# PorousMediaSimulation/openLBMPM

Measured on AMD Instinct MI355X. Metric: MLUPS (million lattice updates/s), higher is better.
Workload: dtype f64

## Files before the change

### include/lbmpm.h

```cpp
#ifndef LBMPM_H
#define LBMPM_H

#include <stddef.h>
#include <stdint.h>

#ifdef __cplusplus
extern "C" {
#endif

typedef enum lbmpm_status {
    LBMPM_OK = 0,
    LBMPM_ERR_INVALID = -1,
    LBMPM_ERR_HIP = -2,
    LBMPM_ERR_NOMEM = -3,
    LBMPM_ERR_STATE = -4,
    LBMPM_ERR_UNSUPPORTED = -5,
    LBMPM_ERR_TIMEOUT = -6
} lbmpm_status;

const char *lbmpm_last_error(void);
const char *lbmpm_version(void);
int lbmpm_device_count(void);
int lbmpm_hbm_stream_test(int device, int64_t bytes_per_buffer, int reps, double *copy_gbs, double *read_gbs, double *inplace_gbs);

// ... 126 lines not shown
int lbmpm_sc2d_create(const lbmpm_sc2d_config *cfg, const uint8_t *is_domain, lbmpm_sc2d **out);
void lbmpm_sc2d_destroy(lbmpm_sc2d *ctx);
int lbmpm_sc2d_set_pdf(lbmpm_sc2d *ctx, const double *pdf0, const double *pdf1);
int lbmpm_sc2d_set_density(lbmpm_sc2d *ctx, const double *rho0, const double *rho1);
int lbmpm_sc2d_step(lbmpm_sc2d *ctx, int64_t nsteps);
int lbmpm_sc2d_step_timed(lbmpm_sc2d *ctx, int64_t nsteps, double *ms_total, double *ms_dominant);
int lbmpm_sc2d_sync(lbmpm_sc2d *ctx);
int lbmpm_sc2d_enable_diagnostics(lbmpm_sc2d *ctx, int on);
int lbmpm_sc2d_get_field(lbmpm_sc2d *ctx, int field, double *out);
int64_t lbmpm_sc2d_num_fluid_nodes(const lbmpm_sc2d *ctx);
int64_t lbmpm_sc2d_steps_done(const lbmpm_sc2d *ctx);
const char *lbmpm_sc2d_dominant_kernel(const lbmpm_sc2d *ctx);
int64_t lbmpm_sc2d_device_bytes(const lbmpm_sc2d *ctx);

typedef struct lbmpm_rk3d_config {
    int64_t nx, ny, nz_local, nz_global, z_offset;
    double ak_r, ak_b;
    double beta;
    double tau_r, tau_b;
    double solid_phi;
    double inlet_vz_r, inlet_vz_b;
    double outlet_rho_r, outlet_rho_b;
    int32_t device;
    int32_t variant;
    int32_t relaxation;
    int32_t inlet_type;
    double recolor_axis, recolor_diag;
    double inlet_rho_r, inlet_rho_b;
    int32_t outlet_type;
    int32_t reserved;
} lbmpm_rk3d_config;

typedef struct lbmpm_rk3d lbmpm_rk3d;

enum { LBMPM_RK3D_PHI = 0, LBMPM_RK3D_RHO_R = 1, LBMPM_RK3D_RHO_B = 2, LBMPM_RK3D_VX = 3,
       LBMPM_RK3D_VY = 4, LBMPM_RK3D_VZ = 5 };
enum { LBMPM_RK3D_BUF_F_SEND_UP = 0, LBMPM_RK3D_BUF_F_SEND_DOWN = 1,
       LBMPM_RK3D_BUF_F_RECV_FROM_BELOW = 2, LBMPM_RK3D_BUF_F_RECV_FROM_ABOVE = 3,
       LBMPM_RK3D_BUF_PHI_SEND_UP = 4, LBMPM_RK3D_BUF_PHI_SEND_DOWN = 5,
       LBMPM_RK3D_BUF_PHI_RECV_FROM_BELOW = 6, LBMPM_RK3D_BUF_PHI_RECV_FROM_ABOVE = 7 };

int lbmpm_rk3d_create(const lbmpm_rk3d_config *cfg, const uint8_t *is_domain_with_halo, lbmpm_rk3d **out);
void lbmpm_rk3d_destroy(lbmpm_rk3d *ctx);
int lbmpm_rk3d_set_stream(lbmpm_rk3d *ctx, void *hip_stream);
int lbmpm_rk3d_set_density(lbmpm_rk3d *ctx, const double *rho_r, const double *rho_b);
int lbmpm_rk3d_set_macro(lbmpm_rk3d *ctx, const double *rho_r, const double *rho_b, const double *vx, const double *vy, const double *vz);
int lbmpm_rk3d_set_pdf(lbmpm_rk3d *ctx, const double *pdf_r, const double *pdf_b, int post_collision);
int lbmpm_rk3d_get_pdf(lbmpm_rk3d *ctx, double *pdf_r, double *pdf_b);
int lbmpm_rk3d_state_info(const lbmpm_rk3d *ctx, int64_t *out);
int lbmpm_rk3d_get_state(lbmpm_rk3d *ctx, double *state);
int lbmpm_rk3d_set_state(lbmpm_rk3d *ctx, const double *state, int64_t doubles_per_cell, int64_t steps_done, int post_collision);
int lbmpm_rk3d_pack_halo(lbmpm_rk3d *ctx);
int lbmpm_rk3d_unpack_halo(lbmpm_rk3d *ctx, int have_below, int have_above);
int lbmpm_rk3d_phase_field(lbmpm_rk3d *ctx, int with_diagnostics);
int lbmpm_rk3d_collide(lbmpm_rk3d *ctx);
int lbmpm_rk3d_collide_interior(lbmpm_rk3d *ctx);
int lbmpm_rk3d_collide_boundary(lbmpm_rk3d *ctx);
typedef int (*lbmpm_rk3d_exchange_fn)(void *user, int what);
int lbmpm_rk3d_step_slab(lbmpm_rk3d *ctx, int64_t nsteps, int has_below, int has_above, lbmpm_rk3d_exchange_fn exchange,
                         void *user, int timed);
int lbmpm_rk3d_slab_timing(lbmpm_rk3d *ctx, double *out);

enum { LBMPM_TRANSPORT_NONE = 0, LBMPM_TRANSPORT_IPC = 1, LBMPM_TRANSPORT_RCCL = 2 };
#define LBMPM_IPC_BLOB_BYTES 256
#define LBMPM_RCCL_ID_BYTES 128
int lbmpm_rk3d_ipc_init(lbmpm_rk3d *ctx, void *blob_out);
int lbmpm_rk3d_ipc_connect(lbmpm_rk3d *ctx, const void *blob_below, const void *blob_above);
int lbmpm_rccl_unique_id(void *id_out, const char *librccl_path);
int lbmpm_rk3d_rccl_connect(lbmpm_rk3d *ctx, const void *id, int rank, int nranks, const char *librccl_path);
int lbmpm_rk3d_transport_disconnect(lbmpm_rk3d *ctx);
int lbmpm_rk3d_transport_kind(lbmpm_rk3d *ctx, int *value_ops);
int lbmpm_rk3d_halo_exchange(lbmpm_rk3d *ctx);
int lbmpm_rk3d_ipc_release_waits(lbmpm_rk3d *ctx);
int lbmpm_rk3d_transport_probe(lbmpm_rk3d *ctx, int rounds);
int lbmpm_rk3d_transport_probe_result(lbmpm_rk3d *ctx, int64_t *mismatches);
int lbmpm_transport_selftest(int kind, int device, int64_t bytes, const char *librccl_path);
int lbmpm_rk3d_step(lbmpm_rk3d *ctx, int64_t nsteps);
int lbmpm_rk3d_step_timed(lbmpm_rk3d *ctx, int64_t nsteps, double *ms_total, double *ms_dominant);
int lbmpm_rk3d_sync(lbmpm_rk3d *ctx);
int lbmpm_rk3d_sync_deadline(lbmpm_rk3d *ctx, double seconds);
int lbmpm_rk3d_buffer(lbmpm_rk3d *ctx, int which, void **device_ptr, int64_t *bytes);
int lbmpm_rk3d_get_field(lbmpm_rk3d *ctx, int field, double *out);
int lbmpm_rk3d_storage_info(lbmpm_rk3d *ctx, int64_t *out);
int lbmpm_rk3d_debug_trace(lbmpm_rk3d *ctx, unsigned long long *out, int64_t nblocks);
int lbmpm_rk3d_debug_plane(lbmpm_rk3d *ctx, int comp, int zl, double *out);
int64_t lbmpm_rk3d_num_fluid_nodes(const lbmpm_rk3d *ctx);
int64_t lbmpm_rk3d_steps_done(const lbmpm_rk3d *ctx);
const char *lbmpm_rk3d_dominant_kernel(const lbmpm_rk3d *ctx);
int64_t lbmpm_rk3d_device_bytes(const lbmpm_rk3d *ctx);

typedef struct lbmpm_rk3dcsf_config {
    int64_t nx, ny, nz;
    double surface_tension;
    double contact_angle_deg;
    double beta, delta;
    double tau_r, tau_b;
    double inlet_velocity_z;
    double inlet_rho_r, inlet_rho_b;
    double outlet_rho_total;
    int32_t wetting_type;
    int32_t tau_type;
    int32_t relaxation;
    int32_t inlet_type;
    int32_t outlet_type;
    int32_t device;
    int32_t variant;
    double mrt_rates[6];
    double bulk_epsilon;
    int32_t ghost_lo, ghost_hi;
    int64_t slab_z0, global_nz;
} lbmpm_rk3dcsf_config;

typedef struct lbmpm_rk3dcsf lbmpm_rk3dcsf;

typedef enum lbmpm_rk3dcsf_field {
    LBMPM_RK3DCSF_PDF_R = 0, LBMPM_RK3DCSF_PDF_B = 1, LBMPM_RK3DCSF_RHO_R = 2, LBMPM_RK3DCSF_RHO_B = 3,
    LBMPM_RK3DCSF_VX = 4, LBMPM_RK3DCSF_VY = 5, LBMPM_RK3DCSF_VZ = 6,
    LBMPM_RK3DCSF_PHI = 7,
    LBMPM_RK3DCSF_GX = 8, LBMPM_RK3DCSF_GY = 9, LBMPM_RK3DCSF_GZ = 10,
    LBMPM_RK3DCSF_FX = 11, LBMPM_RK3DCSF_FY = 12, LBMPM_RK3DCSF_FZ = 13,
    LBMPM_RK3DCSF_K = 14,
    LBMPM_RK3DCSF_NSX = 15, LBMPM_RK3DCSF_NSY = 16, LBMPM_RK3DCSF_NSZ = 17,
    LBMPM_RK3DCSF_KIND = 18,
    LBMPM_RK3DCSF_REC_PDF_R = 30, LBMPM_RK3DCSF_REC_PDF_B = 31, LBMPM_RK3DCSF_REC_RHO_R = 32, LBMPM_RK3DCSF_REC_RHO_B = 33,
    LBMPM_RK3DCSF_REC_VX = 34, LBMPM_RK3DCSF_REC_VY = 35, LBMPM_RK3DCSF_REC_VZ = 36, LBMPM_RK3DCSF_REC_PHI = 37
} lbmpm_rk3dcsf_field;

int lbmpm_rk3dcsf_create(const lbmpm_rk3dcsf_config *cfg, const uint8_t *is_domain, lbmpm_rk3dcsf **out);
void lbmpm_rk3dcsf_destroy(lbmpm_rk3dcsf *ctx);
int lbmpm_rk3dcsf_set_macro(lbmpm_rk3dcsf *ctx, const double *rho_r, const double *rho_b, const double *vx, const double *vy, const double *vz);
int lbmpm_rk3dcsf_set_pdf(lbmpm_rk3dcsf *ctx, const double *pdf_r, const double *pdf_b, const double *fx, const double *fy, const double *fz);
int lbmpm_rk3dcsf_step(lbmpm_rk3dcsf *ctx, int64_t nsteps);
enum { LBMPM_CSF_MSG_PDF = 0, LBMPM_CSF_MSG_PHI = 1, LBMPM_CSF_MSG_NORMAL = 2 };
int lbmpm_rk3dcsf_stage(lbmpm_rk3dcsf *ctx, int stage);
int64_t lbmpm_rk3dcsf_face_doubles(const lbmpm_rk3dcsf *ctx, int msg, int face);
int64_t lbmpm_rk3dcsf_face_doubles_in(const lbmpm_rk3dcsf *ctx, int msg, int face);
int lbmpm_rk3dcsf_face_pack(lbmpm_rk3dcsf *ctx, int msg, int face, double *device_buffer);
int lbmpm_rk3dcsf_face_unpack(lbmpm_rk3dcsf *ctx, int msg, int face, const double *device_buffer);
int lbmpm_rk3dcsf_face_copy(lbmpm_rk3dcsf *src, int src_face, lbmpm_rk3dcsf *dst, int msg);
int lbmpm_rk3dcsf_step_timed(lbmpm_rk3dcsf *ctx, int64_t nsteps, double *ms_total, double *ms_dominant);
int lbmpm_rk3dcsf_sync(lbmpm_rk3dcsf *ctx);
int lbmpm_rk3dcsf_enable_diagnostics(lbmpm_rk3dcsf *ctx, int on);
int lbmpm_rk3dcsf_get_field(lbmpm_rk3dcsf *ctx, int field, double *out);
int64_t lbmpm_rk3dcsf_num_fluid_nodes(const lbmpm_rk3dcsf *ctx);
int64_t lbmpm_rk3dcsf_num_wetting_solids(const lbmpm_rk3dcsf *ctx);
int64_t lbmpm_rk3dcsf_bulk_cells(lbmpm_rk3dcsf *ctx);
int64_t lbmpm_rk3dcsf_steps_done(const lbmpm_rk3dcsf *ctx);
int64_t lbmpm_rk3dcsf_device_bytes(const lbmpm_rk3dcsf *ctx);
const char *lbmpm_rk3dcsf_dominant_kernel(const lbmpm_rk3dcsf *ctx);

typedef struct lbmpm_tracer3d_config {
    int32_t num_tracers;
    double diffusion_x[4];
    double diffusion_y[4];
    double diffusion_z[4];
    double diffusion_xy, diffusion_yx;
    double diffusion_xz, diffusion_zx;
    double diffusion_yz, diffusion_zy;
    double beta_interface[4];
    double criteria_rho;
    double inlet_concentration[4];
    int32_t dirichlet_inlet;
    int32_t free_outlet;
    double reaction_rate;
    double diffusion_j[4];
} lbmpm_tracer3d_config;
// ... 24 lines not shown
```

### openlbmpm_amd/_lib.py

```python
import ctypes as C
import os

_PKG = os.path.dirname(os.path.abspath(__file__))
LIB_PATH = os.environ.get("LBMPM_LIBRARY") or os.path.join(_PKG, "liblbmpm_hip.so")

F64P = C.POINTER(C.c_double)
U8P = C.POINTER(C.c_uint8)
I64P = C.POINTER(C.c_int64)


class LbmpmError(RuntimeError):

    def __init__(self, msg, status=None):
        super().__init__(msg)
        self.status = status


OK, ERR_INVALID, ERR_HIP, ERR_NOMEM, ERR_STATE, ERR_UNSUPPORTED, ERR_TIMEOUT = 0, -1, -2, -3, -4, -5, -6


class RK2DConfig(C.Structure):
    _fields_ = [("nx", C.c_int64), ("ny", C.c_int64),
                ("surface_tension", C.c_double), ("contact_angle_deg", C.c_double),
                ("wetting_type", C.c_int32),
# ... 56 lines not shown

EXCHANGE_FN = C.CFUNCTYPE(C.c_int, C.c_void_p, C.c_int)
IPC_BLOB_BYTES, RCCL_ID_BYTES = 256, 128
TRANSPORT_NONE, TRANSPORT_IPC, TRANSPORT_RCCL = 0, 1, 2

_lib = None

_SIGNATURES = {
    "lbmpm_last_error": (C.c_char_p, []),
    "lbmpm_version": (C.c_char_p, []),
    "lbmpm_device_count": (C.c_int, []),
    "lbmpm_rk2d_create": (C.c_int, [C.POINTER(RK2DConfig), U8P, C.POINTER(C.c_void_p)]),
    "lbmpm_rk2d_destroy": (None, [C.c_void_p]),
    "lbmpm_rk2d_set_pdf": (C.c_int, [C.c_void_p, F64P, F64P]),
    "lbmpm_rk2d_set_macro": (C.c_int, [C.c_void_p, F64P, F64P, F64P, F64P]),
    "lbmpm_rk2d_step": (C.c_int, [C.c_void_p, C.c_int64]),
    "lbmpm_rk2d_step_timed": (C.c_int, [C.c_void_p, C.c_int64, F64P, F64P]),
    "lbmpm_rk2d_sync": (C.c_int, [C.c_void_p]),
    "lbmpm_rk2d_enable_diagnostics": (C.c_int, [C.c_void_p, C.c_int]),
    "lbmpm_rk2d_set_stream": (C.c_int, [C.c_void_p, C.c_void_p]),
    "lbmpm_rk2d_get_field": (C.c_int, [C.c_void_p, C.c_int, F64P]),
    "lbmpm_rk2d_num_fluid_nodes": (C.c_int64, [C.c_void_p]),
    "lbmpm_rk2d_steps_done": (C.c_int64, [C.c_void_p]),
    "lbmpm_rk2d_dominant_kernel": (C.c_char_p, [C.c_void_p]),
    "lbmpm_rk2d_device_bytes": (C.c_int64, [C.c_void_p]),
    "lbmpm_rk2d_tracer_configure": (C.c_int, [C.c_void_p, C.POINTER(TracerConfig)]),
    "lbmpm_rk2d_set_perturbation": (C.c_int, [C.c_void_p, C.POINTER(RK2DPerturbation)]),
    "lbmpm_rk2d_tracer_set_concentration": (C.c_int, [C.c_void_p, C.c_int, F64P]),
    "lbmpm_rk2d_tracer_get_concentration": (C.c_int, [C.c_void_p, C.c_int, F64P]),
    "lbmpm_sc2d_create": (C.c_int, [C.POINTER(SC2DConfig), U8P, C.POINTER(C.c_void_p)]),
    "lbmpm_sc2d_destroy": (None, [C.c_void_p]),
    "lbmpm_sc2d_set_pdf": (C.c_int, [C.c_void_p, F64P, F64P]),
    "lbmpm_sc2d_set_density": (C.c_int, [C.c_void_p, F64P, F64P]),
    "lbmpm_sc2d_step": (C.c_int, [C.c_void_p, C.c_int64]),
    "lbmpm_sc2d_step_timed": (C.c_int, [C.c_void_p, C.c_int64, F64P, F64P]),
    "lbmpm_sc2d_sync": (C.c_int, [C.c_void_p]),
    "lbmpm_sc2d_enable_diagnostics": (C.c_int, [C.c_void_p, C.c_int]),
    "lbmpm_sc2d_get_field": (C.c_int, [C.c_void_p, C.c_int, F64P]),
    "lbmpm_sc2d_num_fluid_nodes": (C.c_int64, [C.c_void_p]),
    "lbmpm_sc2d_steps_done": (C.c_int64, [C.c_void_p]),
    "lbmpm_sc2d_dominant_kernel": (C.c_char_p, [C.c_void_p]),
    "lbmpm_sc2d_device_bytes": (C.c_int64, [C.c_void_p]),
    "lbmpm_rk3d_create": (C.c_int, [C.POINTER(RK3DConfig), U8P, C.POINTER(C.c_void_p)]),
    "lbmpm_rk3d_destroy": (None, [C.c_void_p]),
    "lbmpm_rk3d_set_stream": (C.c_int, [C.c_void_p, C.c_void_p]),
    "lbmpm_rk3d_set_density": (C.c_int, [C.c_void_p, F64P, F64P]),
    "lbmpm_rk3d_set_macro": (C.c_int, [C.c_void_p, F64P, F64P, F64P, F64P, F64P]),
    "lbmpm_rk3d_set_pdf": (C.c_int, [C.c_void_p, F64P, F64P, C.c_int]),
    "lbmpm_rk3d_get_pdf": (C.c_int, [C.c_void_p, F64P, F64P]),
    "lbmpm_rk3d_state_info": (C.c_int, [C.c_void_p, I64P]),
    "lbmpm_rk3d_get_state": (C.c_int, [C.c_void_p, F64P]),
    "lbmpm_rk3d_set_state": (C.c_int, [C.c_void_p, F64P, C.c_int64, C.c_int64, C.c_int]),
    "lbmpm_rk3d_pack_halo": (C.c_int, [C.c_void_p]),
    "lbmpm_rk3d_unpack_halo": (C.c_int, [C.c_void_p, C.c_int, C.c_int]),
    "lbmpm_rk3d_phase_field": (C.c_int, [C.c_void_p, C.c_int]),
    "lbmpm_rk3d_collide": (C.c_int, [C.c_void_p]),
    "lbmpm_rk3d_collide_interior": (C.c_int, [C.c_void_p]),
    "lbmpm_hbm_stream_test": (C.c_int, [C.c_int, C.c_int64, C.c_int, C.POINTER(C.c_double), C.POINTER(C.c_double), C.POINTER(C.c_double)]),
    "lbmpm_rk3d_collide_boundary": (C.c_int, [C.c_void_p]),
    "lbmpm_rk3d_step_slab": (C.c_int, [C.c_void_p, C.c_int64, C.c_int, C.c_int, C.c_void_p, C.c_void_p, C.c_int]),
    "lbmpm_rk3d_slab_timing": (C.c_int, [C.c_void_p, F64P]),
    "lbmpm_rk3d_ipc_init": (C.c_int, [C.c_void_p, C.c_void_p]),
    "lbmpm_rk3d_ipc_connect": (C.c_int, [C.c_void_p, C.c_void_p, C.c_void_p]),
    "lbmpm_rccl_unique_id": (C.c_int, [C.c_void_p, C.c_char_p]),
    "lbmpm_rk3d_rccl_connect": (C.c_int, [C.c_void_p, C.c_void_p, C.c_int, C.c_int, C.c_char_p]),
    "lbmpm_rk3d_transport_disconnect": (C.c_int, [C.c_void_p]),
    "lbmpm_rk3d_transport_kind": (C.c_int, [C.c_void_p, C.POINTER(C.c_int)]),
    "lbmpm_rk3d_halo_exchange": (C.c_int, [C.c_void_p]),
    "lbmpm_rk3d_ipc_release_waits": (C.c_int, [C.c_void_p]),
    "lbmpm_rk3d_transport_probe": (C.c_int, [C.c_void_p, C.c_int]),
    "lbmpm_rk3d_transport_probe_result": (C.c_int, [C.c_void_p, I64P]),
    "lbmpm_transport_selftest": (C.c_int, [C.c_int, C.c_int, C.c_int64, C.c_char_p]),
    "lbmpm_rk3d_step": (C.c_int, [C.c_void_p, C.c_int64]),
    "lbmpm_rk3d_step_timed": (C.c_int, [C.c_void_p, C.c_int64, F64P, F64P]),
    "lbmpm_rk3d_sync": (C.c_int, [C.c_void_p]),
    "lbmpm_rk3d_sync_deadline": (C.c_int, [C.c_void_p, C.c_double]),
    "lbmpm_rk3d_buffer": (C.c_int, [C.c_void_p, C.c_int, C.POINTER(C.c_void_p), I64P]),
    "lbmpm_rk3d_get_field": (C.c_int, [C.c_void_p, C.c_int, F64P]),
    "lbmpm_rk3d_num_fluid_nodes": (C.c_int64, [C.c_void_p]),
    "lbmpm_rk3d_steps_done": (C.c_int64, [C.c_void_p]),
    "lbmpm_rk3d_dominant_kernel": (C.c_char_p, [C.c_void_p]),
    "lbmpm_rk3d_device_bytes": (C.c_int64, [C.c_void_p]),
    "lbmpm_rk3d_storage_info": (C.c_int, [C.c_void_p, I64P]),
    "lbmpm_rk3d_debug_trace": (C.c_int, [C.c_void_p, C.c_void_p, C.c_int64]),
    "lbmpm_rk3d_debug_plane": (C.c_int, [C.c_void_p, C.c_int, C.c_int, F64P]),
    "lbmpm_rk3dcsf_create": (C.c_int, [C.POINTER(RK3DCSFConfig), U8P, C.POINTER(C.c_void_p)]),
    "lbmpm_rk3dcsf_destroy": (None, [C.c_void_p]),
    "lbmpm_rk3dcsf_set_macro": (C.c_int, [C.c_void_p, F64P, F64P, F64P, F64P, F64P]),
    "lbmpm_rk3dcsf_set_pdf": (C.c_int, [C.c_void_p, F64P, F64P, F64P, F64P, F64P]),
    "lbmpm_rk3dcsf_step": (C.c_int, [C.c_void_p, C.c_int64]),
    "lbmpm_rk3dcsf_step_timed": (C.c_int, [C.c_void_p, C.c_int64, F64P, F64P]),
    "lbmpm_rk3dcsf_stage": (C.c_int, [C.c_void_p, C.c_int]),
    "lbmpm_rk3dcsf_face_doubles": (C.c_int64, [C.c_void_p, C.c_int, C.c_int]),
    "lbmpm_rk3dcsf_face_doubles_in": (C.c_int64, [C.c_void_p, C.c_int, C.c_int]),
    "lbmpm_rk3dcsf_face_pack": (C.c_int, [C.c_void_p, C.c_int, C.c_int, C.c_void_p]),
    "lbmpm_rk3dcsf_face_unpack": (C.c_int, [C.c_void_p, C.c_int, C.c_int, C.c_void_p]),
    "lbmpm_rk3dcsf_face_copy": (C.c_int, [C.c_void_p, C.c_int, C.c_void_p, C.c_int]),
    "lbmpm_rk3dcsf_sync": (C.c_int, [C.c_void_p]),
    "lbmpm_rk3dcsf_enable_diagnostics": (C.c_int, [C.c_void_p, C.c_int]),
    "lbmpm_rk3dcsf_get_field": (C.c_int, [C.c_void_p, C.c_int, F64P]),
    "lbmpm_rk3dcsf_num_fluid_nodes": (C.c_int64, [C.c_void_p]),
    "lbmpm_rk3dcsf_num_wetting_solids": (C.c_int64, [C.c_void_p]),
    "lbmpm_rk3dcsf_bulk_cells": (C.c_int64, [C.c_void_p]),
    "lbmpm_rk3dcsf_steps_done": (C.c_int64, [C.c_void_p]),
    "lbmpm_rk3dcsf_device_bytes": (C.c_int64, [C.c_void_p]),
    "lbmpm_rk3dcsf_dominant_kernel": (C.c_char_p, [C.c_void_p]),
    "lbmpm_rk3dcsf_tracer_configure": (C.c_int, [C.c_void_p, C.POINTER(Tracer3DConfig)]),
    "lbmpm_rk3dcsf_tracer_configure_slab": (C.c_int, [C.c_void_p, C.POINTER(Tracer3DConfig)]),
    "lbmpm_rk3dcsf_tracer_set_concentration": (C.c_int, [C.c_void_p, C.c_int, F64P]),
    "lbmpm_rk3dcsf_tracer_get_concentration": (C.c_int, [C.c_void_p, C.c_int, F64P]),
    "lbmpm_rk3dcsf_tracer_get_pdf": (C.c_int, [C.c_void_p, C.c_int, F64P]),
    "lbmpm_rk3dcsf_tracer_set_pdf": (C.c_int, [C.c_void_p, C.c_int, F64P]),
    "lbmpm_rk3dcsf_ipc_init": (C.c_int, [C.c_void_p, C.c_void_p]),
    "lbmpm_rk3dcsf_ipc_connect": (C.c_int, [C.c_void_p, C.c_void_p, C.c_void_p]),
    "lbmpm_rk3dcsf_rccl_connect": (C.c_int, [C.c_void_p, C.c_void_p, C.c_int, C.c_int, C.c_char_p]),
    "lbmpm_rk3dcsf_transport_disconnect": (C.c_int, [C.c_void_p]),
    "lbmpm_rk3dcsf_transport_kind": (C.c_int, [C.c_void_p, C.POINTER(C.c_int)]),
    "lbmpm_rk3dcsf_transport_probe": (C.c_int, [C.c_void_p, C.c_int]),
    "lbmpm_rk3dcsf_transport_probe_result": (C.c_int, [C.c_void_p, I64P]),
    "lbmpm_rk3dcsf_ipc_release_waits": (C.c_int, [C.c_void_p]),
    "lbmpm_rk3dcsf_step_slab": (C.c_int, [C.c_void_p, C.c_int64, C.c_int]),
    "lbmpm_rk3dcsf_slab_timing": (C.c_int, [C.c_void_p, F64P]),
    "lbmpm_rk3dcsf_sync_deadline": (C.c_int, [C.c_void_p, C.c_double]),
}


def _share_hip_runtime_with_torch():
    import importlib.util
    import sys
    if "torch" in sys.modules:
        return
    try:
        spec = importlib.util.find_spec("torch")
    except (ImportError, ValueError):
        spec = None
    if spec is None or not spec.origin:
        return
    cand = os.path.join(os.path.dirname(spec.origin), "lib", "libamdhip64.so")
    if os.path.exists(cand):
        try:
            C.CDLL(cand, mode=C.RTLD_GLOBAL)
        except OSError:
            pass


_loaded = {}


def _load(path):
    if path in _loaded:
        return _loaded[path]
    if not os.path.exists(path):
        raise LbmpmError("%s is missing: the HIP library is the only compute path "
                         "(no CPU fallback). Build it: python -m openlbmpm_amd.build" % path)
    _share_hip_runtime_with_torch()
    try:
        L = C.CDLL(path)
    except OSError as e:
        raise LbmpmError("cannot load %s: %s" % (path, e))
    for name, (res, args) in _SIGNATURES.items():
        fn = getattr(L, name)
        fn.restype = res
        fn.argtypes = args
    _loaded[path] = L
    return L

# ... 19 lines not shown
```

### openlbmpm_amd/csrc/rk3d.hip

```cpp
#include <type_traits>
#include "lbmpm_common.h"
#include "d2q9_device.h"

#include <cmath>
#include <cstdlib>
#include <cstring>

namespace {

using lbmpm::set_error;
using lbmpm_dev::wrapi;

constexpr int Q = 19;
#define LBMPM_D3Q19_CX {0, 1, -1, 0, 0, 0, 0, 1, -1, 1, -1, 1, -1, 1, -1, 0, 0, 0, 0}
#define LBMPM_D3Q19_CY {0, 0, 0, 1, -1, 0, 0, 1, -1, -1, 1, 0, 0, 0, 0, 1, -1, 1, -1}
#define LBMPM_D3Q19_CZ {0, 0, 0, 0, 0, 1, -1, 0, 0, 0, 0, 1, -1, -1, 1, 1, -1, -1, 1}
#define LBMPM_D3Q19_OPP {0, 2, 1, 4, 3, 6, 5, 8, 7, 10, 9, 12, 11, 14, 13, 16, 15, 18, 17}
__device__ __forceinline__ constexpr double wq(int i) { return i == 0 ? 1. / 3. : (i < 7 ? 1. / 18. : 1. / 36.); }
__device__ __forceinline__ constexpr double bq(int i) { return i == 0 ? -1. / 3. : (i < 7 ? 1. / 18. : 1. / 36.); }

typedef unsigned u32x4 __attribute__((ext_vector_type(4)));

struct RK3Dev {
    int nx, ny, nzl, pitch;
    unsigned plane_bytes;
    size_t plane2, vol;
    int z0, nzg;
    const uint8_t *flags;
    const uint32_t *solidnbr;
    const double *fin;
    double *fout;
    double *phi;
    double *diag;
    double ak, beta, cR, cB, solidPhi, vzR, vzB, rhoOutR, rhoOutB;
    double rcA, rcD;
    int first, fill;
    int mrt;
    const u32x4 *seg;
    const u32x4 *seg2;
    const unsigned long long *pstart;
    int nseg;
    const uint32_t *pur_in;
    uint32_t *pur_out;
#ifdef LBMPM_DEV
    unsigned long long *trace;
#endif
    int halo_lo;
    int conv;
    int inletP;
};

struct Cell { unsigned o[3][3]; };

__device__ __forceinline__ Cell make_cell(const RK3Dev &p, int x, int y)
{
    Cell c;
    const int xs[3] = {wrapi(x - 1, p.nx), x, wrapi(x + 1, p.nx)}, ys[3] = {wrapi(y - 1, p.ny), y, wrapi(y + 1, p.ny)};
#pragma unroll
    for (int a = 0; a < 3; ++a)
#pragma unroll
        for (int b = 0; b < 3; ++b) c.o[a][b] = (unsigned)(ys[a] * p.pitch + xs[b]) * 8u;
    return c;
}

__device__ __forceinline__ Cell fresh(const Cell &c)
{
    Cell r = c;
#pragma unroll
    for (int a = 0; a < 3; ++a)
#pragma unroll
        for (int b = 0; b < 3; ++b) asm volatile("" : "+v"(r.o[a][b]));
    return r;
}

__device__ __forceinline__ const char *plane_ptr(const double *f, const RK3Dev &p, int zl)
{
    return reinterpret_cast<const char *>(f) + (size_t)zl * (2 * Q) * p.plane_bytes;
}
__device__ __forceinline__ double ldg(const char *uniform_base, unsigned off) { return *reinterpret_cast<const double *>(uniform_base + off); }
__device__ __forceinline__ void stg(char *uniform_base, unsigned off, double v) { *reinterpret_cast<double *>(uniform_base + off) = v; }

template <bool FIRST>
__device__ __forceinline__ void pull3(const RK3Dev &p, const Cell &c, int zl, unsigned sn, double fR[Q], double fB[Q])
{
    constexpr int CX[Q] = LBMPM_D3Q19_CX, CY[Q] = LBMPM_D3Q19_CY, CZ[Q] = LBMPM_D3Q19_CZ, OPP[Q] = LBMPM_D3Q19_OPP;
    const unsigned pb = p.plane_bytes, own = c.o[1][1];
    const char *red = plane_ptr(p.fin, p, zl - 1), *blue = red + (size_t)Q * pb;
    fR[0] = ldg(red, (unsigned)(2 * Q) * pb + own);
    fB[0] = ldg(blue, (unsigned)(2 * Q) * pb + own);
#pragma unroll
    for (int i = 1; i < Q; ++i) {
        const unsigned up = (unsigned)((1 - CZ[i]) * 2 * Q + i) * pb + c.o[1 - CY[i]][1 - CX[i]];
        const unsigned back = (unsigned)(2 * Q + OPP[i]) * pb + own;
        const unsigned s = FIRST ? (unsigned)(2 * Q + i) * pb + own : (((sn >> (OPP[i] - 1)) & 1u) ? back : up);
        fR[i] = ldg(red, s);
        fB[i] = ldg(blue, s);
    }
}

__device__ __forceinline__ unsigned load_meta(const RK3Dev &p, int zl, unsigned own)
{
    return *reinterpret_cast<const unsigned *>(reinterpret_cast<const char *>(p.solidnbr + (size_t)zl * p.plane2) + (own >> 1));
}

__device__ __forceinline__ int source_plane(const RK3Dev &p, int zl)
{
    const int zg = p.z0 + zl - 1;
    return zg == p.nzg - 1 ? zl - 1 : (zg == 0 ? zl + 1 : zl);
}

__device__ __forceinline__ int source_plane_x(const RK3Dev &p, int zl)
{
    const int zg = p.z0 + zl - 1;
    if (p.conv && zg <= 2) return zl + (3 - zg);
    return source_plane(p, zl);
}

__device__ __forceinline__ double sum19(const double f[Q])
{
    double r = 0.;
#pragma unroll
    for (int i = 0; i < Q; ++i) r += f[i];
    return r;
}

__device__ __forceinline__ double zouhe_inlet(double uz, double f[Q])
{
    const double s0 = f[0] + f[1] + f[2] + f[3] + f[4] + f[7] + f[8] + f[9] + f[10];
    const double sp = f[5] + f[11] + f[14] + f[15] + f[18];
    const double rho = (s0 + 2. * sp) / (1. + uz);
    const double Nx = 0.5 * ((f[1] + f[7] + f[9]) - (f[2] + f[8] + f[10]));
    const double Ny = 0.5 * ((f[3] + f[7] + f[10]) - (f[4] + f[8] + f[9]));
// ... 793 lines not shown
            send_up[(size_t)(c * 5 + j) * p.plane2 + k] = top[(size_t)(c * Q + UP[j]) * p.plane2 + k];
            send_dn[(size_t)(c * 5 + j) * p.plane2 + k] = bot[(size_t)(c * Q + DN[j]) * p.plane2 + k];
        }
}

__global__ void rk3d_unpack(RK3Dev p, double *f, const double *recv_from_below, const double *recv_from_above,
                            int have_below, int have_above)
{
    constexpr int UP[5] = {5, 11, 14, 15, 18}, DN[5] = {6, 12, 13, 16, 17};
    const size_t k = (size_t)blockIdx.x * blockDim.x + threadIdx.x;
    if (k >= p.plane2) return;
    double *lo = f, *hi = f + (size_t)(p.nzl + 1) * 2 * Q * p.plane2;
    for (int c = 0; c < 2; ++c)
        for (int j = 0; j < 5; ++j) {
            if (have_below) lo[(size_t)(c * Q + UP[j]) * p.plane2 + k] = recv_from_below[(size_t)(c * 5 + j) * p.plane2 + k];
            if (have_above) hi[(size_t)(c * Q + DN[j]) * p.plane2 + k] = recv_from_above[(size_t)(c * 5 + j) * p.plane2 + k];
        }
}

__global__ void rk3d_init_rest(RK3Dev p, const double *rho_r, const double *rho_b, double *f)
{
    const int x = blockIdx.x * BX3 + threadIdx.x, y = blockIdx.y * BY3 + threadIdx.y, zl = blockIdx.z + 1;
    if (x >= p.nx || y >= p.ny) return;
    const size_t cell = (size_t)y * p.pitch + x;
    const bool fluid = p.flags[(size_t)zl * p.plane2 + cell] & 1;
    const size_t s = ((size_t)(zl - 1) * p.ny + y) * p.nx + x;
    const double a = fluid ? rho_r[s] : 0., b = fluid ? rho_b[s] : 0.;
    double *pl = f + (size_t)zl * 2 * Q * p.plane2;
    for (int i = 0; i < Q; ++i) {
        pl[(size_t)i * p.plane2 + cell] = wq(i) * a;
        pl[(size_t)(Q + i) * p.plane2 + cell] = wq(i) * b;
    }
}

__global__ void rk3d_init_phi(RK3Dev p, double *phi)
{
    const size_t k = (size_t)blockIdx.x * blockDim.x + threadIdx.x;
    if (k < p.vol && !(p.flags[k] & 1)) phi[k] = p.solidPhi;
}

__global__ void rk3d_setup_solidnbr(RK3Dev p, uint32_t *solidnbr)
{
    constexpr int CX[Q] = LBMPM_D3Q19_CX, CY[Q] = LBMPM_D3Q19_CY, CZ[Q] = LBMPM_D3Q19_CZ;
    const int x = blockIdx.x * BX3 + threadIdx.x, y = blockIdx.y * BY3 + threadIdx.y, zl = blockIdx.z;
    if (x >= p.nx || y >= p.ny) return;
    unsigned b = 0;
    for (int i = 1; i < Q; ++i) {
        const int zn = zl + CZ[i];
        bool fluid = false;
        if (zn >= 0 && zn <= p.nzl + 1)
            fluid = p.flags[(size_t)zn * p.plane2 + (size_t)wrapi(y + CY[i], p.ny) * p.pitch + wrapi(x + CX[i], p.nx)] & 1;
        if (!fluid) b |= 1u << (i - 1);
    }
    if (p.flags[(size_t)zl * p.plane2 + (size_t)y * p.pitch + x] & 1) b |= 1u << 31;
    solidnbr[(size_t)zl * p.plane2 + (size_t)y * p.pitch + x] = b;
}

#include "rk3dq.h"
#include "rk3d_state.h"

}

#include "rk3d_transport.h"

struct lbmpm_rk3d {
    lbmpm_rk3d_config cfg;
    int nx, ny, nzl, pitch;
    size_t plane2, vol;
    int64_t nfluid = 0;
    hipStream_t stream = nullptr;
    bool own_stream = false;
    uint8_t *flags = nullptr;
    uint32_t *solidnbr = nullptr;
    double *fA = nullptr, *fB = nullptr, *phi = nullptr, *diag = nullptr;
    uint32_t *purA = nullptr, *purB = nullptr;
    double *send_up = nullptr, *send_dn = nullptr, *recv_below = nullptr, *recv_above = nullptr;
    std::vector<uint8_t> h_domain;
    bool conv = false;
    int conv_lo = 0;
    bool compact = false;
    bool q23 = false;
    unsigned long long *trace = nullptr;
    unsigned *slotq = nullptr;
    unsigned slot_launches = 0;
    unsigned long long *probe_bad = nullptr;
    slabtx::Transport tx;
    bool halo_valid = false;
    int dbg = 0;
    int nseg = 0;
    size_t ncells = 0;
    unsigned long long *pstart = nullptr;
    uint32_t *seg = nullptr, *seg2 = nullptr;
    std::vector<unsigned long long> h_pstart;
    std::vector<uint8_t> h_rowpop;
    bool streamed = false;
    int variant = 0, tile = 0, chunk_len = 32, fill = 16;
    bool chunk_auto = false;
    int ncu = 256;
    int boundary = 2;
    hipStream_t aux = nullptr;
    hipEvent_t ev_dep = nullptr, ev_done = nullptr;
    bool interior_pending = false;
    int64_t steps = 0, bytes = 0;
    lbmpm::EventPool slab_pool;
    int64_t slab_timed_steps = 0;
    unsigned long long *beat_host = nullptr, *beat_dev = nullptr;
    hipStream_t wd_stream = nullptr;
    int64_t observed_at = -1;
    lbmpm::EventPool pool;
};

namespace {

RK3Dev make_dev(const lbmpm_rk3d *c)
{
    RK3Dev p{};
    p.nx = c->nx; p.ny = c->ny; p.nzl = c->nzl; p.pitch = c->pitch; p.plane2 = c->plane2; p.vol = c->vol;
    p.plane_bytes = (unsigned)(c->plane2 * sizeof(double));
    p.seg = reinterpret_cast<const u32x4 *>(c->seg); p.seg2 = reinterpret_cast<const u32x4 *>(c->seg2); p.pstart = c->pstart; p.nseg = c->nseg;
    p.z0 = (int)c->cfg.z_offset; p.nzg = (int)c->cfg.nz_global;
    p.flags = c->flags; p.solidnbr = c->solidnbr; p.fin = c->fA; p.fout = c->fB; p.phi = c->phi; p.diag = nullptr;
    p.ak = (c->cfg.ak_r + c->cfg.ak_b) * 0.5; p.beta = c->cfg.beta; p.cR = 1. / (2. * (c->cfg.tau_r - 0.5)); p.cB = 1. / (2. * (c->cfg.tau_b - 0.5));
    p.solidPhi = c->cfg.solid_phi; p.vzR = c->cfg.inlet_vz_r; p.vzB = c->cfg.inlet_vz_b;
    p.rhoOutR = c->cfg.outlet_rho_r; p.rhoOutB = c->cfg.outlet_rho_b;
    p.conv = c->conv ? 1 : 0;
    p.halo_lo = 0;
    p.inletP = c->cfg.inlet_type == LBMPM_INLET_PRESSURE ? 1 : 0;
    if (p.inletP) { p.vzR = c->cfg.inlet_rho_r; p.vzB = c->cfg.inlet_rho_b; }
    p.rcA = c->cfg.beta * (c->cfg.recolor_axis > 0. ? c->cfg.recolor_axis : 1. / 18.);
    p.rcD = c->cfg.beta * (c->cfg.recolor_diag > 0. ? c->cfg.recolor_diag : (1. / 36.) * 0.70710678118654752440);
    p.first = c->streamed ? 0 : 1;
    p.fill = c->fill;
    p.mrt = c->cfg.relaxation;
#ifdef LBMPM_DEV
    p.trace = c->trace;
#endif
    p.pur_in = c->purA; p.pur_out = c->purB;
    return p;
}

template <typename T>
int dev_alloc(lbmpm_rk3d *c, T **ptr, size_t count)
{
    void *v = nullptr;
    hipError_t e = hipMalloc(&v, count * sizeof(T));
    if (e != hipSuccess) { set_error("hipMalloc(%zu bytes) failed: %s", count * sizeof(T), hipGetErrorString(e)); return LBMPM_ERR_NOMEM; }
    e = hipMemsetAsync(v, 0, count * sizeof(T), c->stream);
    if (e != hipSuccess) { set_error("hipMemsetAsync failed: %s", hipGetErrorString(e)); return LBMPM_ERR_HIP; }
    *ptr = static_cast<T *>(v);
    c->bytes += (int64_t)(count * sizeof(T));
    return LBMPM_OK;
}

dim3 grid3(const lbmpm_rk3d *c, int planes) { return dim3((c->nx + BX3 - 1) / BX3, (c->ny + BY3 - 1) / BY3, planes); }

}

extern "C" int lbmpm_rk3d_create(const lbmpm_rk3d_config *cfg, const uint8_t *is_domain_with_halo, lbmpm_rk3d **out)
{
    LBMPM_REQUIRE(cfg && is_domain_with_halo && out, "lbmpm_rk3d_create: null argument");
    LBMPM_REQUIRE(cfg->nx >= 4 && cfg->ny >= 4 && cfg->nz_local >= 2 && cfg->nz_global >= 8,
                  "lbmpm_rk3d_create: domain %lld x %lld x %lld(local) out of range", (long long)cfg->nx,
                  (long long)cfg->ny, (long long)cfg->nz_local);
    LBMPM_REQUIRE(cfg->z_offset >= 0 && cfg->z_offset + cfg->nz_local <= cfg->nz_global, "slab [%lld, %lld) outside 0..%lld",
                  (long long)cfg->z_offset, (long long)(cfg->z_offset + cfg->nz_local), (long long)cfg->nz_global);
    LBMPM_REQUIRE(cfg->tau_r > 0.5 && cfg->tau_b > 0.5, "TauR/TauB must exceed 0.5");
    LBMPM_REQUIRE(cfg->outlet_rho_r > 0. && cfg->outlet_rho_b > 0., "densityRL/densityBL must be positive (the Zou-He outlet divides by them; the shipped ini uses 1e-8 for the absent colour)");
    LBMPM_REQUIRE((double)cfg->nx * cfg->ny * (cfg->nz_local + 2) < 2.0e9, "slab too large for 32-bit plane indices");
    LBMPM_REQUIRE((double)(cfg->nx + 31) * cfg->ny * 8.0 * 6 * Q < 4.0e9, "xy plane too large: 114 planes must fit 32-bit byte offsets (about 4.3M cells per plane)");
    int variant = cfg->variant, tile = 0, chunk_len = 32, fill = 16;
    bool chunk_fixed = false;
    if (const char *e = getenv("LBMPM_RK3D_VARIANT")) variant = atoi(e);
#ifdef LBMPM_DEV
    if (const char *e = getenv("LBMPM_RK3D_TILE")) tile = atoi(e);
    if (const char *e = getenv("LBMPM_RK3D_CHUNK")) { chunk_len = atoi(e) > 0 ? atoi(e) : 32; chunk_fixed = true; }
    if (const char *e = getenv("LBMPM_RK3D_FILL")) fill = atoi(e);
#endif
    LBMPM_REQUIRE(variant == 0 || variant == 1, "lbmpm_rk3d_create: variant must be 0 (fused) or 1 (split)");
    LBMPM_REQUIRE(cfg->relaxation == 0 || cfg->relaxation == 1, "lbmpm_rk3d_create: relaxation must be 0 (SRT) or 1 (MRT)");
    LBMPM_REQUIRE(cfg->outlet_type == LBMPM_OUTLET_PRESSURE || cfg->outlet_type == LBMPM_OUTLET_CONVECTIVE, "lbmpm_rk3d_create: outlet_type must be LBMPM_OUTLET_PRESSURE or LBMPM_OUTLET_CONVECTIVE");
    if (cfg->outlet_type == LBMPM_OUTLET_CONVECTIVE) {
        LBMPM_REQUIRE(cfg->nz_global >= 8 && (cfg->z_offset == 0 ? cfg->nz_local >= 6 : cfg->z_offset >= 6),
                      "lbmpm_rk3d_create: the convective outlet needs nz >= 8 and the lattice's bottom slab to own the planes 0 .. 5 at least (slab [%lld, %lld))",
                      (long long)cfg->z_offset, (long long)(cfg->z_offset + cfg->nz_local));
        LBMPM_REQUIRE(cfg->variant == 0 && !getenv("LBMPM_RK3D_VARIANT"), "lbmpm_rk3d_create: the convective outlet runs the fused schedule only");
        if (cfg->z_offset == 0) {
            const size_t hp = (size_t)cfg->nx * cfg->ny;
            for (int z = 2; z <= 4; ++z)
                LBMPM_REQUIRE(memcmp(is_domain_with_halo + hp, is_domain_with_halo + (size_t)z * hp, hp) == 0,
                              "lbmpm_rk3d_create: the convective outlet copies plane 3 onto the planes 2, 1, 0: their masks must coincide (plane %d differs from plane 0)", z - 1);
        }
    }
    LBMPM_REQUIRE(cfg->inlet_type == LBMPM_INLET_VELOCITY || (cfg->inlet_type == LBMPM_INLET_PRESSURE && cfg->inlet_rho_r > 0. && cfg->inlet_rho_b > 0.),
                  "lbmpm_rk3d_create: inlet_type must be LBMPM_INLET_VELOCITY or LBMPM_INLET_PRESSURE with positive densityRH / densityBH (the Zou-He pressure plane divides by them)");
    LBMPM_REQUIRE(cfg->recolor_axis >= 0. && cfg->recolor_diag >= 0. && cfg->recolor_axis < 1. && cfg->recolor_diag < 1.,
                  "lbmpm_rk3d_create: recolor_axis / recolor_diag must be 0 (the model's weights) or a weight in (0, 1)");
    LBMPM_REQUIRE(fill == 0 || fill == 4 || fill == 8 || fill == 16 || fill == 32 || fill == 64,
                  "LBMPM_RK3D_FILL must be 0 or a power of two <= 64");
    LBMPM_HIP_TRY(hipSetDevice(cfg->device));
    lbmpm_rk3d *c = new (std::nothrow) lbmpm_rk3d();
    if (!c) { set_error("out of host memory"); return LBMPM_ERR_NOMEM; }
    c->cfg = *cfg;
    c->nx = (int)cfg->nx; c->ny = (int)cfg->ny; c->nzl = (int)cfg->nz_local;
    c->variant = variant; c->tile = tile; c->chunk_len = chunk_len; c->fill = fill;
#ifdef LBMPM_DEV
    if (const char *e = getenv("LBMPM_RK3D_BOUNDARY")) c->boundary = atoi(e) >= 2 ? atoi(e) : 2;
#endif
    c->conv = cfg->outlet_type == LBMPM_OUTLET_CONVECTIVE;
    c->conv_lo = c->conv && cfg->z_offset == 0 ? 3 : 0;
    c->compact = variant == 0;
    if (const char *e = getenv("LBMPM_RK3D_LAYOUT")) if (!strcmp(e, "dense")) c->compact = false;
    c->q23 = c->compact && c->tile == 0;
    if (const char *e = getenv("LBMPM_RK3D_STORAGE")) if (atoi(e) == 38) c->q23 = false;
    if (!c->q23 && c->nx % 64 != 0) c->compact = false;
    if (c->conv && !c->q23) c->compact = false;
    if (c->q23 && (c->nx > 32767 || c->ny > 32767)) {
        set_error("lbmpm_rk3d_create: nx and ny must not exceed 32767 (%d x %d)", c->nx, c->ny);
        delete c;
        return LBMPM_ERR_INVALID;
    }
#ifdef LBMPM_DEV
    if (const char *e = getenv("LBMPM_RK3D_DBG")) c->dbg = atoi(e);
#endif
    c->chunk_auto = c->q23 && !chunk_fixed;
    if (c->chunk_auto) { c->chunk_len = 64; (void)hipDeviceGetAttribute(&c->ncu, hipDeviceAttributeMultiprocessorCount, cfg->device); if (c->ncu <= 0) c->ncu = 256; }
#ifdef LBMPM_DEV
    if (c->q23 && getenv("LBMPM_RK3D_TRACE")) { (void)hipMalloc(reinterpret_cast<void **>(&c->trace), (size_t)1 << 22); (void)hipMemset(c->trace, 0, (size_t)1 << 22); }
#endif
    c->pitch = (c->nx + 31) / 32 * 32;
    c->plane2 = (size_t)c->pitch * c->ny;
    c->vol = c->plane2 * (size_t)(c->nzl + 2);
    const size_t hp = (size_t)c->nx * c->ny;
    c->h_domain.assign(is_domain_with_halo + hp, is_domain_with_halo + hp * (size_t)(c->nzl + 1));
    std::vector<uint8_t> hflags(c->vol, 0);
    for (int z = 0; z < c->nzl + 2; ++z)
        for (int y = 0; y < c->ny; ++y)
            for (int x = 0; x < c->nx; ++x) {
                const uint8_t v = is_domain_with_halo[(size_t)z * hp + (size_t)y * c->nx + x] == 1 ? 1 : 0;
                hflags[(size_t)z * c->plane2 + (size_t)y * c->pitch + x] = v;
                if (z >= 1 && z <= c->nzl) c->nfluid += v;
            }
    if (c->nfluid == 0) { set_error("lbmpm_rk3d_create: the slab has no fluid node (is_domain == 1 marks fluid); cut the lattice elsewhere"); delete c; return LBMPM_ERR_INVALID; }
    {
        hipError_t e = hipStreamCreateWithFlags(&c->stream, hipStreamNonBlocking);
        if (e != hipSuccess) { set_error("hipStreamCreate failed: %s", hipGetErrorString(e)); delete c; return LBMPM_ERR_HIP; }
        c->own_stream = true;
    }
    int rc = LBMPM_OK;
#define TRY_RC(e) do { rc = (e); if (rc != LBMPM_OK) { lbmpm_rk3d_destroy(c); return rc; } } while (0)
    TRY_RC(dev_alloc(c, &c->flags, c->vol));
    TRY_RC(dev_alloc(c, &c->solidnbr, c->vol));
    std::vector<uint32_t> hseg, hseg2;
    if (c->compact) {
        c->nseg = (c->nx + 63) / 64;
        const int ns = c->nseg;
        auto sx0 = [&](int sg) { return seg_x0(sg, c->nx, ns); };
        const size_t rows = (size_t)(c->nzl + 2) * c->ny;
        hseg.assign(rows * ns * 4, 0u);
        hseg2.assign(rows * ns * 4, 0u);
        c->h_pstart.assign(c->nzl + 3, 0ull);
        c->h_rowpop.assign(rows * ns, 0);
        unsigned long long total = 0;
        std::vector<unsigned long long> m((size_t)c->ny * ns);
        std::vector<unsigned> first((size_t)c->ny * ns);
        for (int z = 0; z < c->nzl + 2; ++z) {
            c->h_pstart[z] = total;
            for (int y = 0; y < c->ny; ++y)
                for (int sg = 0; sg < ns; ++sg) {
                    const uint8_t *fl = hflags.data() + (size_t)z * c->plane2 + (size_t)y * c->pitch + sx0(sg);
                    unsigned long long w = 0;
                    for (int b = 0; b < sx0(sg + 1) - sx0(sg); ++b)
                        if (fl[b]) w |= 1ull << b;
                    m[(size_t)y * ns + sg] = w;
                }
            unsigned j = 0;
            for (int y0 = 0; y0 < c->ny; y0 += TILE_ROWS)
                for (int sg = 0; sg < ns; ++sg) {
                    int last = -1;
                    for (int y = y0; y < y0 + TILE_ROWS && y < c->ny; ++y) {
                        first[(size_t)y * ns + sg] = j;
                        j += (unsigned)__builtin_popcountll(m[(size_t)y * ns + sg]);
                        last = y;
                    }
                    const unsigned lc = c->q23 ? (unsigned)QLINE : 8u;
                    const unsigned pad = (lc - (j % lc)) % lc;
                    hseg[(((size_t)z * c->ny + last) * ns + sg) * 4 + 3] = pad << 2;
                    j += pad;
                }
            if (j > 0 && ((size_t)j * (c->q23 ? 8u : 16u)) % 16384u == 0) j += 73u * 16u;
            for (int y = 0; y < c->ny; ++y)
                for (int sg = 0; sg < ns; ++sg) {
                    const size_t r = ((size_t)z * c->ny + y) * ns + sg;
                    const int sl = sg > 0 ? sg - 1 : ns - 1, sr = sg + 1 < ns ? sg + 1 : 0;
                    const unsigned long long ml = m[(size_t)y * ns + sl], mr = m[(size_t)y * ns + sr];
                    c->h_rowpop[r] = (uint8_t)__builtin_popcountll(m[(size_t)y * ns + sg]);
                    hseg[r * 4 + 0] = (uint32_t)m[(size_t)y * ns + sg];
                    hseg[r * 4 + 1] = (uint32_t)(m[(size_t)y * ns + sg] >> 32);
                    hseg[r * 4 + 2] = first[(size_t)y * ns + sg];
                    const int wl = sx0(sl + 1) - sx0(sl), wd = sx0(sg + 1) - sx0(sg);
                    hseg[r * 4 + 3] |= (uint32_t)((ml >> (wl - 1)) & 1ull) | ((uint32_t)(mr & 1ull) << 1) | ((uint32_t)(64 - wd) << 8);
                    hseg2[r * 4 + 0] = first[(size_t)y * ns + sl] + (unsigned)__builtin_popcountll(ml) - 1u;
                    hseg2[r * 4 + 1] = first[(size_t)y * ns + sr];
                }
            total += j;
        }
        c->h_pstart[c->nzl + 2] = total;
        c->ncells = (size_t)total;
        TRY_RC(dev_alloc(c, &c->seg, hseg.size()));
        TRY_RC(dev_alloc(c, &c->seg2, hseg2.size()));
        TRY_RC(dev_alloc(c, &c->pstart, c->h_pstart.size()));
    }
    const size_t fcount = c->q23 ? (size_t)QS * (c->ncells + 2) : (c->compact ? 2 * Q * (c->ncells + 1) : 2 * Q * c->vol);
    TRY_RC(dev_alloc(c, &c->fA, fcount));
    TRY_RC(dev_alloc(c, &c->fB, fcount));
    if (c->q23) {
        bool by_xcc = true;
#ifdef LBMPM_DEV
        if (getenv("LBMPM_RK3D_XCC") && atoi(getenv("LBMPM_RK3D_XCC")) == 0) by_xcc = false;
#endif
        if (by_xcc) TRY_RC(dev_alloc(c, &c->slotq, 2 * 4096 * 8));
        LBMPM_REQUIRE((size_t)(c->nzl + 2) * c->ny * c->nseg < ((size_t)1 << 31), "rk3d: more than 2^31 row segments in one slab");
        TRY_RC(dev_alloc(c, &c->purA, (size_t)(c->nzl + 2) * c->ny * c->nseg));
        TRY_RC(dev_alloc(c, &c->purB, (size_t)(c->nzl + 2) * c->ny * c->nseg));
    }
    TRY_RC(dev_alloc(c, &c->phi, c->vol));
    size_t max_cnt = c->plane2;
    if (c->compact) for (int z = 0; z < c->nzl + 2; ++z) max_cnt = std::max(max_cnt, (size_t)(c->h_pstart[z + 1] - c->h_pstart[z]));
    const size_t face_doubles = (c->q23 ? FACE_DOUBLES + 1 : 10) * max_cnt;
    TRY_RC(dev_alloc(c, &c->send_up, face_doubles));
    TRY_RC(dev_alloc(c, &c->send_dn, face_doubles));
    TRY_RC(dev_alloc(c, &c->recv_below, face_doubles));
    TRY_RC(dev_alloc(c, &c->recv_above, face_doubles));
#undef TRY_RC
    hipError_t e = hipMemcpyAsync(c->flags, hflags.data(), c->vol, hipMemcpyHostToDevice, c->stream);
    if (e == hipSuccess && c->compact) e = hipMemcpyAsync(c->seg, hseg.data(), hseg.size() * sizeof(hseg[0]), hipMemcpyHostToDevice, c->stream);
    if (e == hipSuccess && c->compact) e = hipMemcpyAsync(c->seg2, hseg2.data(), hseg2.size() * sizeof(hseg2[0]), hipMemcpyHostToDevice, c->stream);
    if (e == hipSuccess && c->compact) e = hipMemcpyAsync(c->pstart, c->h_pstart.data(), c->h_pstart.size() * sizeof(c->h_pstart[0]), hipMemcpyHostToDevice, c->stream);
    if (e == hipSuccess) e = hipStreamSynchronize(c->stream);
    if (e != hipSuccess) { set_error("flags upload failed: %s", hipGetErrorString(e)); lbmpm_rk3d_destroy(c); return LBMPM_ERR_HIP; }
    RK3Dev p = make_dev(c);
    rk3d_setup_solidnbr<<<grid3(c, c->nzl + 2), dim3(BX3, BY3), 0, c->stream>>>(p, c->solidnbr);
    rk3d_init_phi<<<dim3((unsigned)((c->vol + 255) / 256)), dim3(256), 0, c->stream>>>(p, c->phi);
    e = hipStreamSynchronize(c->stream);
    if (e == hipSuccess) e = hipGetLastError();
    if (e != hipSuccess) { set_error("set-up kernel failed: %s", hipGetErrorString(e)); lbmpm_rk3d_destroy(c); return LBMPM_ERR_HIP; }
    *out = c;
    return LBMPM_OK;
}

extern "C" void lbmpm_rk3d_destroy(lbmpm_rk3d *c)
{
    if (!c) return;
    (void)hipSetDevice(c->cfg.device);
    if (c->stream) (void)hipStreamSynchronize(c->stream);
    if (c->aux) (void)hipStreamSynchronize(c->aux);
    c->tx.disconnect();
    if (c->probe_bad) (void)hipFree(c->probe_bad);
    if (c->beat_host) (void)hipHostFree(c->beat_host);
    if (c->wd_stream) (void)hipStreamDestroy(c->wd_stream);
    for (void *ptr : {(void *)c->seg, (void *)c->seg2, (void *)c->pstart, (void *)c->flags, (void *)c->solidnbr, (void *)c->fA, (void *)c->fB, (void *)c->purA, (void *)c->purB, (void *)c->trace, (void *)c->slotq, (void *)c->phi, (void *)c->diag,
                      (void *)c->send_up, (void *)c->send_dn, (void *)c->recv_below, (void *)c->recv_above})
        if (ptr) (void)hipFree(ptr);
    c->pool.destroy();
    c->slab_pool.destroy();
    if (c->aux) { (void)hipStreamDestroy(c->aux); (void)hipEventDestroy(c->ev_dep); (void)hipEventDestroy(c->ev_done); }
    if (c->own_stream && c->stream) (void)hipStreamDestroy(c->stream);
    delete c;
}

extern "C" int lbmpm_rk3d_set_stream(lbmpm_rk3d *c, void *hip_stream)
{
    LBMPM_REQUIRE(c, "null context");
    LBMPM_HIP_TRY(hipStreamSynchronize(c->stream));
    if (hip_stream == nullptr) {
        if (!c->own_stream) { LBMPM_HIP_TRY(hipStreamCreateWithFlags(&c->stream, hipStreamNonBlocking)); c->own_stream = true; }
        return LBMPM_OK;
    }
    if (c->own_stream) { (void)hipStreamDestroy(c->stream); c->own_stream = false; }
    c->stream = static_cast<hipStream_t>(hip_stream);
    return LBMPM_OK;
}

extern "C" int lbmpm_rk3d_set_density(lbmpm_rk3d *c, const double *rho_r, const double *rho_b)
{
    LBMPM_REQUIRE(c && rho_r && rho_b, "lbmpm_rk3d_set_density: null argument");
    LBMPM_HIP_TRY(hipSetDevice(c->cfg.device));
    const size_t n = (size_t)c->nx * c->ny * c->nzl;
    const size_t fbytes = (c->q23 ? (size_t)QS * (c->ncells + 2) : (c->compact ? 2 * Q * (c->ncells + 1) : 2 * Q * c->vol)) * sizeof(double);
    double *stage = nullptr;
    LBMPM_HIP_TRY(hipMalloc(reinterpret_cast<void **>(&stage), 2 * n * sizeof(double)));
    hipError_t e = hipMemcpyAsync(stage, rho_r, n * sizeof(double), hipMemcpyHostToDevice, c->stream);
    if (e == hipSuccess) e = hipMemcpyAsync(stage + n, rho_b, n * sizeof(double), hipMemcpyHostToDevice, c->stream);
    if (e == hipSuccess) e = hipMemsetAsync(c->fA, 0, fbytes, c->stream);
    if (e == hipSuccess) e = hipMemsetAsync(c->fB, 0, fbytes, c->stream);
    if (e == hipSuccess) {
        RK3Dev p = make_dev(c);
        if (c->q23) {
            const size_t pbytes = (size_t)(c->nzl + 2) * c->ny * c->nseg * sizeof(uint32_t);
            e = hipMemsetAsync(c->purA, 0xff, pbytes, c->stream);
            rk3dq_init_rest<<<dim3(c->nseg, (c->ny + BY3 - 1) / BY3, c->nzl), dim3(BX3, BY3), 0, c->stream>>>(p, stage, stage + n, c->fA, c->purA);
            if (e == hipSuccess) e = hipMemcpyAsync(c->fB, c->fA, fbytes, hipMemcpyDeviceToDevice, c->stream);
            if (e == hipSuccess) e = hipMemcpyAsync(c->purB, c->purA, pbytes, hipMemcpyDeviceToDevice, c->stream);
        }
        else if (c->compact) rk3dc_init_rest<<<grid3(c, c->nzl), dim3(BX3, BY3), 0, c->stream>>>(p, stage, stage + n, c->fA);
        else rk3d_init_rest<<<grid3(c, c->nzl), dim3(BX3, BY3), 0, c->stream>>>(p, stage, stage + n, c->fA);
        e = hipGetLastError();
    }
    if (e == hipSuccess) e = hipStreamSynchronize(c->stream);
    (void)hipFree(stage);
    if (e != hipSuccess) { set_error("lbmpm_rk3d_set_density: %s", hipGetErrorString(e)); return LBMPM_ERR_HIP; }
    LBMPM_HIP_TRY(hipStreamSynchronize(c->stream));
    c->streamed = false;
    c->halo_valid = false;
    c->steps = 0;
    c->observed_at = -1;
    return LBMPM_OK;
}

namespace {
template <int MODE>
void launch_state_io(lbmpm_rk3d *c, const RK3Dev &p, double *f, int zl0, int planes, double *a, double *b)
{
    const dim3 block(BX3, BY3);
    const unsigned gy = (unsigned)((c->ny + BY3 - 1) / BY3);
    if (c->q23) rk3d_state_io<ST_Q23, MODE><<<dim3(c->nseg, gy, planes), block, 0, c->stream>>>(p, f, zl0, a, b);
    else if (c->compact) rk3d_state_io<ST_C38, MODE><<<dim3(c->nseg, gy, planes), block, 0, c->stream>>>(p, f, zl0, a, b);
    else rk3d_state_io<ST_DENSE, MODE><<<dim3((c->nx + 63) / 64, gy, planes), block, 0, c->stream>>>(p, f, zl0, a, b);
}

int state_width(const lbmpm_rk3d *c) { return c->q23 ? QS : 2 * Q; }
size_t state_fbytes(const lbmpm_rk3d *c) { return (c->q23 ? (size_t)QS * (c->ncells + 2) : (c->compact ? 2 * Q * (c->ncells + 1) : 2 * Q * c->vol)) * sizeof(double); }

template <int MODE>
int state_transfer(lbmpm_rk3d *c, double *ha, int wa, double *hb, int wb, const double *const *m)
{
    constexpr bool GET = MODE == IO_GET_STATE || MODE == IO_GET_PDF;
    LBMPM_REQUIRE(!c->interior_pending, "state transfer inside a step: finish it with lbmpm_rk3d_collide_boundary first");
    LBMPM_HIP_TRY(hipSetDevice(c->cfg.device));
    LBMPM_HIP_TRY(hipStreamSynchronize(c->stream));
    if (c->aux) LBMPM_HIP_TRY(hipStreamSynchronize(c->aux));
    const size_t pcells = (size_t)c->nx * c->ny;
    const int per = MODE == IO_SET_MACRO ? 5 : wa + wb;
    int batch = (int)(((size_t)256 << 20) / (pcells * (size_t)per * sizeof(double)));
// ... 143 lines not shown
    const dim3 grid((unsigned)((c->plane2 + threads - 1) / threads));
    if (c->compact) rk3dc_unpack<<<grid, dim3(threads), 0, c->stream>>>(p, c->fA, c->recv_below, c->recv_above, have_below, have_above);
    else rk3d_unpack<<<grid, dim3(threads), 0, c->stream>>>(p, c->fA, c->recv_below, c->recv_above, have_below, have_above);
    LBMPM_HIP_TRY(hipGetLastError());
    return LBMPM_OK;
}

extern "C" int lbmpm_rk3d_phase_field(lbmpm_rk3d *c, int with_diagnostics)
{
    LBMPM_REQUIRE(c, "null context");
    LBMPM_HIP_TRY(hipSetDevice(c->cfg.device));
    if (with_diagnostics && !c->diag) { const int rc = dev_alloc(c, &c->diag, 5 * c->vol); if (rc) return rc; }
    RK3Dev p = make_dev(c);
    p.diag = with_diagnostics ? c->diag : nullptr;
    auto k1 = [&](int planes, int zl0) {
        if (c->q23) rk3dq_phase_field<<<dim3(c->nseg, (c->ny + BY3 - 1) / BY3, planes), dim3(BX3, BY3), 0, c->stream>>>(p, zl0);
        else if (c->compact) rk3dc_phase_field<<<dim3(c->nseg, (c->ny + BY3 - 1) / BY3, planes), dim3(BX3, BY3), 0, c->stream>>>(p, zl0);
        else rk3d_phase_field<<<grid3(c, planes), dim3(BX3, BY3), 0, c->stream>>>(p, zl0);
    };
    if (with_diagnostics) c->observed_at = c->steps;
    if (c->variant == 1 || with_diagnostics) k1(c->nzl, 1);
    else if (c->q23) {  }
    else {
        if (c->cfg.z_offset > 0) k1(1, 1);
        if (c->cfg.z_offset + c->cfg.nz_local < c->cfg.nz_global && (c->nzl > 1 || c->cfg.z_offset == 0)) k1(1, c->nzl);
    }
    LBMPM_HIP_TRY(hipGetLastError());
    return LBMPM_OK;
}

namespace {
template <typename F>
void dispatch2(bool a, bool b, F &&f)
{
    if (a) { if (b) f(std::true_type{}, std::true_type{}); else f(std::true_type{}, std::false_type{}); }
    else   { if (b) f(std::false_type{}, std::true_type{}); else f(std::false_type{}, std::false_type{}); }
}

template <int TX, int TY>
void launch_fused(lbmpm_rk3d *c, const RK3Dev &p, hipStream_t st, int z_first, int z_last)
{
    const int tilesX = (c->nx + TX - 1) / TX, tilesY = (c->ny + TY - 1) / TY, rpx = (tilesY + 7) / 8;
    const int nchunks = (z_last - z_first + 1 + c->chunk_len - 1) / c->chunk_len;
    const dim3 grid((unsigned)(8 * tilesX * rpx * nchunks)), block(TX * TY);
    auto go = [&](auto first, auto mrt) {
        rk3d_fused<TX, TY, decltype(first)::value, decltype(mrt)::value><<<grid, block, 0, st>>>(p, tilesX, tilesY, rpx, c->chunk_len, z_first, z_last);
    };
    dispatch2(p.first != 0, p.mrt != 0, go);
}

template <int TY>
void launch_fused_c(lbmpm_rk3d *c, const RK3Dev &p, hipStream_t st, int z_first, int z_last)
{
    const int tilesX = c->nseg, tilesY = (c->ny + TY - 1) / TY, rpx = (tilesY + 7) / 8;
    const int nchunks = (z_last - z_first + 1 + c->chunk_len - 1) / c->chunk_len;
    const dim3 grid((unsigned)(8 * tilesX * rpx * nchunks)), block(64 * TY);
    auto go = [&](auto first, auto mrt) {
        rk3dc_fused<TY, decltype(first)::value, decltype(mrt)::value><<<grid, block, 0, st>>>(p, tilesX, tilesY, rpx, c->chunk_len, z_first, z_last);
    };
    dispatch2(p.first != 0, p.mrt != 0, go);
}

int chunk_planes(const lbmpm_rk3d *c, int n)
{
    if (!c->chunk_auto) return c->chunk_len;
    const int tiles = c->nseg * ((c->ny + 7) / 8);
    const int want = (4 * c->ncu + tiles - 1) / tiles;
    int len = (n + want - 1) / want;
    int minlen = 64;
    while (minlen > 8 && tiles * ((n + minlen - 1) / minlen) < c->ncu) minlen /= 2;
    if (len < minlen) len = minlen;
    const int nch = (n + len - 1) / len;
    return nch > 0 ? (n + nch - 1) / nch : 64;
}

void launch_q23(lbmpm_rk3d *c, const RK3Dev &p, hipStream_t st, int z_first, int z_last, int z_first2, int z_last2)
{
    const int tilesX = c->nseg, tilesY = (c->ny + 7) / 8, rpx = (tilesY + 7) / 8;
    const int n1 = z_last - z_first + 1, n2 = z_last2 >= z_first2 ? z_last2 - z_first2 + 1 : 0;
    const int chunk_len = chunk_planes(c, n1 > n2 ? n1 : n2);
    const int nchunks1 = (n1 + chunk_len - 1) / chunk_len;
    const int nchunks2 = n2 > 0 ? (n2 + chunk_len - 1) / chunk_len : 0;
    const dim3 grid((unsigned)(8 * tilesX * rpx * (nchunks1 + nchunks2))), block(512);
    unsigned *q = nullptr;
    if (c->slotq) {
        const unsigned n = c->slot_launches++, ring = (n / 4096u) & 1u, i = n % 4096u;
        if (i == 2048u) (void)hipMemsetAsync(c->slotq + (size_t)(ring ^ 1u) * 4096u * 8u, 0, 4096u * 8u * sizeof(unsigned), st);
        q = c->slotq + ((size_t)ring * 4096u + i) * 8u;
    }
    auto go = [&](auto first, auto mrt) {
        constexpr bool F = decltype(first)::value, M = decltype(mrt)::value;
        auto launch = [&](auto ragged, auto pin) {
            rk3dq_fused<F, M, decltype(ragged)::value, decltype(pin)::value><<<grid, block, 0, st>>>(p, tilesX, tilesY, rpx, chunk_len, z_first, z_last,
                                                                                                     nchunks1, z_first2, z_last2, q);
        };
        dispatch2(c->nx % 64 != 0, p.inletP != 0, launch);
    };
    dispatch2(p.first != 0, p.mrt != 0, go);
}

void launch_step_range(lbmpm_rk3d *c, const RK3Dev &p, hipStream_t st, int z_first, int z_last)
{
    if (z_last < z_first) return;
    if (c->q23 && c->conv_lo > 0) {
        const int zs = c->conv_lo + 1;
        if (z_last < zs) return;
        if (z_first <= zs) {
            const dim3 block(BX3, BY3);
            const unsigned gy = (unsigned)((c->ny + BY3 - 1) / BY3);
            RK3Dev q = p;
            q.diag = nullptr;
            rk3dq_phase_field<<<dim3(c->nseg, gy, 1), block, 0, st>>>(q, zs);
            rk3dq_conv_phi<<<dim3((unsigned)((c->plane2 + 255) / 256)), dim3(256), 0, st>>>(q, zs);
            RK3Dev m = p;
            m.halo_lo = c->conv_lo;
            launch_q23(c, m, st, zs, z_last, 1, 0);
            dispatch2(p.first != 0, p.mrt != 0, [&](auto first, auto mrt) {
                rk3dq_conv_collide<decltype(first)::value, decltype(mrt)::value><<<dim3(c->nseg, gy, 2), block, 0, st>>>(p, zs);
            });
            return;
        }
    }
    if (c->q23) { launch_q23(c, p, st, z_first, z_last, 1, 0); return; }
    if (c->compact) {
        if (c->tile == 1) launch_fused_c<4>(c, p, st, z_first, z_last);
        else launch_fused_c<8>(c, p, st, z_first, z_last);
        return;
    }
    if (c->tile == 1) launch_fused<64, 4>(c, p, st, z_first, z_last);
    else if (c->tile == 2) launch_fused<32, 8>(c, p, st, z_first, z_last);
    else launch_fused<64, 8>(c, p, st, z_first, z_last);
}

void finish_step(lbmpm_rk3d *c)
{
    std::swap(c->fA, c->fB);
    std::swap(c->purA, c->purB);
    c->streamed = true;
    c->steps += 1;
    c->halo_valid = false;
}
}

extern "C" int lbmpm_rk3d_collide(lbmpm_rk3d *c)
{
    LBMPM_REQUIRE(c, "null context");
    LBMPM_REQUIRE(!c->interior_pending, "lbmpm_rk3d_collide after lbmpm_rk3d_collide_interior: finish the step with lbmpm_rk3d_collide_boundary");
    RK3Dev p = make_dev(c);
    if (c->variant == 1) {
        if (p.mrt) rk3d_collide<true><<<grid3(c, c->nzl), dim3(BX3, BY3), 0, c->stream>>>(p);
        else rk3d_collide<false><<<grid3(c, c->nzl), dim3(BX3, BY3), 0, c->stream>>>(p);
    }
    else launch_step_range(c, p, c->stream, 1, c->nzl);
    LBMPM_HIP_TRY(hipGetLastError());
    finish_step(c);
    return LBMPM_OK;
}

static int collide_interior_ev(lbmpm_rk3d *c, hipEvent_t e0, hipEvent_t e1);
static int collide_boundary_ev(lbmpm_rk3d *c, hipEvent_t e0, hipEvent_t e1);
extern "C" int lbmpm_rk3d_collide_interior(lbmpm_rk3d *c) { return collide_interior_ev(c, nullptr, nullptr); }
extern "C" int lbmpm_rk3d_collide_boundary(lbmpm_rk3d *c) { return collide_boundary_ev(c, nullptr, nullptr); }

static int collide_interior_ev(lbmpm_rk3d *c, hipEvent_t e0, hipEvent_t e1)
{
    LBMPM_REQUIRE(c, "null context");
    LBMPM_REQUIRE(!c->interior_pending, "lbmpm_rk3d_collide_interior called twice in one step");
    const int cb = c->boundary;
    if (c->variant == 1 || c->nzl < 2 * cb + 1) return LBMPM_OK;
    LBMPM_HIP_TRY(hipSetDevice(c->cfg.device));
    if (!c->aux) {
        LBMPM_HIP_TRY(hipStreamCreateWithFlags(&c->aux, hipStreamNonBlocking));
        LBMPM_HIP_TRY(hipEventCreateWithFlags(&c->ev_dep, hipEventDisableTiming));
        LBMPM_HIP_TRY(hipEventCreateWithFlags(&c->ev_done, hipEventDisableTiming));
    }
    LBMPM_HIP_TRY(hipEventRecord(c->ev_dep, c->stream));
    LBMPM_HIP_TRY(hipStreamWaitEvent(c->aux, c->ev_dep, 0));
    RK3Dev p = make_dev(c);
    if (e0) LBMPM_HIP_TRY(hipEventRecord(e0, c->aux));
    launch_step_range(c, p, c->aux, cb + 1, c->nzl - cb);
    LBMPM_HIP_TRY(hipGetLastError());
    if (e1) LBMPM_HIP_TRY(hipEventRecord(e1, c->aux));
    LBMPM_HIP_TRY(hipEventRecord(c->ev_done, c->aux));
    c->interior_pending = true;
    return LBMPM_OK;
}

static int collide_boundary_ev(lbmpm_rk3d *c, hipEvent_t e0, hipEvent_t e1)
{
    LBMPM_REQUIRE(c, "null context");
    if (!c->interior_pending) {
        if (e0) LBMPM_HIP_TRY(hipEventRecord(e0, c->stream));
        const int rc = lbmpm_rk3d_collide(c);
        if (rc == LBMPM_OK && e1) LBMPM_HIP_TRY(hipEventRecord(e1, c->stream));
        return rc;
    }
    const int cb = c->boundary;
    RK3Dev p = make_dev(c);
    if (e0) LBMPM_HIP_TRY(hipEventRecord(e0, c->stream));
    launch_step_range(c, p, c->stream, 1, cb);
    launch_step_range(c, p, c->stream, c->nzl - cb + 1, c->nzl);
    LBMPM_HIP_TRY(hipGetLastError());
    if (e1) LBMPM_HIP_TRY(hipEventRecord(e1, c->stream));
    LBMPM_HIP_TRY(hipStreamWaitEvent(c->stream, c->ev_done, 0));
    c->interior_pending = false;
    finish_step(c);
    return LBMPM_OK;
}

static int tx_shape(lbmpm_rk3d *c)
{
    LBMPM_REQUIRE(c->q23, "the in-library transports move the one-exchange face message of the compact 23-value storage (LBMPM_RK3D_STORAGE, _LAYOUT, _TILE, _VARIANT unset)");
    const bool below = c->cfg.z_offset > 0, above = c->cfg.z_offset + c->cfg.nz_local < c->cfg.nz_global;
    return c->tx.set_shape(c->cfg.device, below, above, (size_t)face_bytes(c, c->nzl), (size_t)face_bytes(c, 1), (size_t)face_bytes(c, 0),
                           (size_t)face_bytes(c, c->nzl + 1));
}

extern "C" int lbmpm_rk3d_ipc_init(lbmpm_rk3d *c, void *blob_out)
{
    LBMPM_REQUIRE(c && blob_out, "lbmpm_rk3d_ipc_init: null argument");
    int rc = tx_shape(c);
    slabtx::IpcBlob b;
    if (rc == LBMPM_OK) rc = c->tx.ipc_alloc(&b);
    if (rc != LBMPM_OK) { c->tx.disconnect(); return rc; }
    memset(blob_out, 0, LBMPM_IPC_BLOB_BYTES);
    memcpy(blob_out, &b, sizeof b);
    return LBMPM_OK;
}

extern "C" int lbmpm_rk3d_ipc_connect(lbmpm_rk3d *c, const void *blob_below, const void *blob_above)
{
    LBMPM_REQUIRE(c && c->tx.kind == LBMPM_TRANSPORT_IPC && !c->tx.connected, "lbmpm_rk3d_ipc_connect: call lbmpm_rk3d_ipc_init first (once)");
    LBMPM_REQUIRE((blob_below != nullptr) == c->tx.has_below && (blob_above != nullptr) == c->tx.has_above,
                  "lbmpm_rk3d_ipc_connect: a blob for exactly the neighbours this slab has (below: %d, above: %d)", (int)c->tx.has_below, (int)c->tx.has_above);
    LBMPM_HIP_TRY(hipSetDevice(c->cfg.device));
    slabtx::IpcBlob b;
    int rc = LBMPM_OK;
    if (blob_below) { memcpy(&b, blob_below, sizeof b); rc = c->tx.ipc_open(0, &b, c->tx.bytes_dn); }
    if (rc == LBMPM_OK && blob_above) { memcpy(&b, blob_above, sizeof b); rc = c->tx.ipc_open(1, &b, c->tx.bytes_up); }
    if (rc != LBMPM_OK) return rc;
    c->tx.connected = true;
    c->halo_valid = false;
    return LBMPM_OK;
}

extern "C" int lbmpm_rccl_unique_id(void *id_out, const char *librccl_path)
{
    LBMPM_REQUIRE(id_out, "lbmpm_rccl_unique_id: null argument");
    slabtx::Rccl r;
    int rc = r.open(librccl_path);
    if (rc != LBMPM_OK) return rc;
    slabtx::Rccl::UniqueId id;
    const int e = r.GetUniqueId(&id);
    if (e != 0) { set_error("ncclGetUniqueId: %s", r.GetErrorString(e)); r.close(); return LBMPM_ERR_HIP; }
    memcpy(id_out, &id, LBMPM_RCCL_ID_BYTES);
    return LBMPM_OK;
}

extern "C" int lbmpm_rk3d_rccl_connect(lbmpm_rk3d *c, const void *id, int rank, int nranks, const char *librccl_path)
{
    LBMPM_REQUIRE(c && id && nranks >= 1 && rank >= 0 && rank < nranks, "lbmpm_rk3d_rccl_connect: bad argument");
    int rc = tx_shape(c);
    if (rc != LBMPM_OK) { c->tx.disconnect(); return rc; }
    if (!((c->tx.has_below ? rank > 0 : true) && (c->tx.has_above ? rank + 1 < nranks : true))) {
        set_error("lbmpm_rk3d_rccl_connect: rank %d of %d has no rank %s it, but the slab has a neighbour there", rank, nranks, c->tx.has_below && rank == 0 ? "below" : "above");
        c->tx.disconnect();
        return LBMPM_ERR_INVALID;
    }
    rc = c->tx.rccl.open(librccl_path);
    if (rc != LBMPM_OK) { c->tx.disconnect(); return rc; }
    slabtx::Rccl::UniqueId uid;
    memcpy(&uid, id, sizeof uid);
    if (hipSetDevice(c->cfg.device) != hipSuccess) { set_error("hipSetDevice(%d) failed", c->cfg.device); c->tx.disconnect(); return LBMPM_ERR_HIP; }
    const int e = c->tx.rccl.CommInitRank(&c->tx.comm, nranks, uid, rank);
    if (e != 0) { set_error("ncclCommInitRank(rank %d of %d): %s", rank, nranks, c->tx.rccl.GetErrorString(e)); c->tx.disconnect(); return LBMPM_ERR_HIP; }
    c->tx.rank = rank; c->tx.nranks = nranks; c->tx.peer_up = rank + 1; c->tx.peer_dn = rank - 1;
    c->tx.kind = LBMPM_TRANSPORT_RCCL; c->tx.connected = true; c->tx.seq = 0;
    c->halo_valid = false;
    return LBMPM_OK;
}

// ... 133 lines not shown
    LBMPM_HIP_TRY(hipSetDevice(c->cfg.device));
    if (!c->tx.has_below && !c->tx.has_above) return LBMPM_OK;
    int rc = lbmpm_rk3d_pack_halo(c);
    if (rc == LBMPM_OK) rc = tx_exchange_unpack(c, make_dev(c), c->fA, c->purA, true);
    if (rc == LBMPM_OK) c->halo_valid = true;
    return rc;
}

extern "C" int lbmpm_rk3d_step_slab(lbmpm_rk3d *c, int64_t nsteps, int has_below, int has_above, lbmpm_rk3d_exchange_fn exchange,
                                    void *user, int timed)
{
    LBMPM_REQUIRE(c && nsteps >= 0, "lbmpm_rk3d_step_slab: bad argument");
    const bool nb = has_below || has_above;
    const bool own_tx = nb && !exchange && c->tx.connected;
    LBMPM_REQUIRE(!nb || exchange || own_tx, "lbmpm_rk3d_step_slab: a slab with neighbours needs an exchange callback or a connected transport");
    LBMPM_REQUIRE(!own_tx || c->q23, "the in-library transports serve the compact 23-value storage");
    LBMPM_REQUIRE((has_below != 0) == (c->cfg.z_offset > 0) && (has_above != 0) == (c->cfg.z_offset + c->cfg.nz_local < c->cfg.nz_global),
                  "lbmpm_rk3d_step_slab: has_below / has_above contradict the slab's position in the lattice");
    LBMPM_HIP_TRY(hipSetDevice(c->cfg.device));
    const int64_t tsteps = timed ? (nsteps < 256 ? nsteps : 256) : 0;
    if (timed) {
        if (c->slab_pool.reserve((size_t)(4 * tsteps)) != LBMPM_OK) { set_error("hipEventCreate failed"); return LBMPM_ERR_HIP; }
        c->slab_pool.reset();
        c->slab_timed_steps = tsteps;
    }
    if (c->q23 && nb) {
        LBMPM_REQUIRE(!c->interior_pending, "lbmpm_rk3d_step_slab: finish the step begun with lbmpm_rk3d_collide_interior first");
        auto fail = [&](int code) {
            if (c->aux) (void)hipStreamSynchronize(c->aux);
            (void)hipStreamSynchronize(c->stream);
            c->halo_valid = false;
            return code;
        };
#define SLAB_HIP_TRY(expr) do { const hipError_t e_ = (expr); if (e_ != hipSuccess) { set_error("%s failed: %s (%s:%d)", #expr, hipGetErrorString(e_), __FILE__, __LINE__); return fail(LBMPM_ERR_HIP); } } while (0)
        if (!c->beat_host) {
            SLAB_HIP_TRY(hipHostMalloc(reinterpret_cast<void **>(&c->beat_host), 64, hipHostMallocMapped));
            *c->beat_host = 0ull;
            SLAB_HIP_TRY(hipHostGetDevicePointer(reinterpret_cast<void **>(&c->beat_dev), c->beat_host, 0));
        }
        if (!c->halo_valid) {
            int rc;
            if (own_tx) rc = lbmpm_rk3d_halo_exchange(c);
            else {
                rc = lbmpm_rk3d_pack_halo(c);
                if (rc == LBMPM_OK && exchange(user, 0) != 0) { set_error("lbmpm_rk3d_step_slab: the exchange callback failed (priming the halo planes)"); rc = LBMPM_ERR_STATE; }
                if (rc == LBMPM_OK) rc = lbmpm_rk3d_unpack_halo(c, has_below, has_above);
            }
            if (rc != LBMPM_OK) return fail(rc);
        }
        if (!c->aux) {
#ifdef LBMPM_DEV
            int reserve = 0, ncu = 0;
            if (const char *e = getenv("LBMPM_RK3D_COMM_CUS")) reserve = atoi(e);
            (void)hipDeviceGetAttribute(&ncu, hipDeviceAttributeMultiprocessorCount, c->cfg.device);
            if (reserve > 0 && ncu >= 64 && reserve < ncu / 2) {
                std::vector<uint32_t> mask((size_t)(ncu + 31) / 32, 0u);
                for (int i = 0; i < ncu - reserve; ++i) mask[(size_t)i / 32] |= 1u << (i % 32);
                if (hipExtStreamCreateWithCUMask(&c->aux, (uint32_t)mask.size(), mask.data()) != hipSuccess) { (void)hipGetLastError(); c->aux = nullptr; }
            }
#endif
            if (!c->aux) SLAB_HIP_TRY(hipStreamCreateWithFlags(&c->aux, hipStreamNonBlocking));
            SLAB_HIP_TRY(hipEventCreateWithFlags(&c->ev_dep, hipEventDisableTiming));
            SLAB_HIP_TRY(hipEventCreateWithFlags(&c->ev_done, hipEventDisableTiming));
        }
        const int cb = c->boundary;
        const bool has_interior = c->nzl >= 2 * cb + 1;
        const dim3 fgrid(c->nseg, (c->ny + BY3 - 1) / BY3, 2), fblock(BX3, BY3);
#ifdef LBMPM_DEV
        const char *sched = getenv("LBMPM_RK3D_SLAB_SCHEDULE");
#else
        const char *sched = nullptr;
#endif
        const bool one_stream = has_interior && !(sched && !strcmp(sched, "split")) && ((sched && !strcmp(sched, "one")) || !own_tx || c->tx.kind != LBMPM_TRANSPORT_RCCL);
        if (one_stream) {
            SLAB_HIP_TRY(hipEventRecord(c->ev_dep, c->stream));
            for (int64_t k = 0; k < nsteps; ++k) {
                hipEvent_t ev[8] = {nullptr, nullptr, nullptr, nullptr, nullptr, nullptr, nullptr, nullptr};
                if (k < tsteps) for (int i = 0; i < 4; ++i) c->slab_pool.take(&ev[2 * i], &ev[2 * i + 1]);
                const RK3Dev p = make_dev(c);
                if (ev[0]) SLAB_HIP_TRY(hipEventRecord(ev[0], c->aux));
                SLAB_HIP_TRY(hipStreamWaitEvent(c->aux, c->ev_dep, 0));
                if (ev[6]) SLAB_HIP_TRY(hipEventRecord(ev[6], c->aux));
                const int zi0 = has_below ? cb + 1 : 1, zi1 = has_above ? c->nzl - cb : c->nzl;
                if (has_below && has_above) launch_q23(c, p, c->aux, 1, cb, c->nzl - cb + 1, c->nzl);
                else if (has_below) launch_q23(c, p, c->aux, 1, cb, 1, 0);
                else launch_q23(c, p, c->aux, c->nzl - cb + 1, c->nzl, 1, 0);
                if (ev[7]) SLAB_HIP_TRY(hipEventRecord(ev[7], c->aux));
                RK3Dev q = p;
                q.fin = c->fB; q.pur_in = c->purB; q.first = 0;
                rk3dq_face_pack<<<fgrid, fblock, 0, c->aux>>>(q, c->send_up, c->send_dn, has_below, has_above);
                SLAB_HIP_TRY(hipEventRecord(c->ev_done, c->aux));
                if (hipGetLastError() != hipSuccess) { set_error("lbmpm_rk3d_step_slab: kernel launch failed"); return fail(LBMPM_ERR_HIP); }
                if (ev[2]) SLAB_HIP_TRY(hipEventRecord(ev[2], c->aux));
                launch_step_range(c, p, c->aux, zi0, zi1);
                if (ev[3]) SLAB_HIP_TRY(hipEventRecord(ev[3], c->aux));
                SLAB_HIP_TRY(hipStreamWaitEvent(c->stream, c->ev_done, 0));
                if (ev[4]) SLAB_HIP_TRY(hipEventRecord(ev[4], c->stream));
                const double *from_below = c->recv_below, *from_above = c->recv_above;
                if (own_tx) { const int rc = c->tx.exchange(c->stream, c->send_up, c->send_dn, &from_below, &from_above); if (rc != LBMPM_OK) return fail(rc); }
                else if (exchange(user, 0) != 0) { set_error("lbmpm_rk3d_step_slab: the exchange callback failed"); return fail(LBMPM_ERR_STATE); }
                rk3dq_face_unpack<<<fgrid, fblock, 0, c->stream>>>(q, c->fB, c->purB, from_below, from_above, has_below, has_above);
                rk3dq_halo_phi<<<fgrid, fblock, 0, c->stream>>>(q, from_below, from_above, has_below, has_above);
                slabtx::launch_flag_store(c->stream, c->beat_dev, (unsigned long long)(c->steps + 1));
                if (ev[5]) SLAB_HIP_TRY(hipEventRecord(ev[5], c->stream));
                SLAB_HIP_TRY(hipEventRecord(c->ev_dep, c->stream));
                if (hipGetLastError() != hipSuccess) { set_error("lbmpm_rk3d_step_slab: kernel launch failed"); return fail(LBMPM_ERR_HIP); }
                finish_step(c);
                c->halo_valid = true;
                if (ev[1]) SLAB_HIP_TRY(hipEventRecord(ev[1], c->aux));
            }
            SLAB_HIP_TRY(hipEventRecord(c->ev_done, c->aux));
            SLAB_HIP_TRY(hipStreamWaitEvent(c->stream, c->ev_done, 0));
            return LBMPM_OK;
        }
        for (int64_t k = 0; k < nsteps; ++k) {
            hipEvent_t ev[8] = {nullptr, nullptr, nullptr, nullptr, nullptr, nullptr, nullptr, nullptr};
            if (k < tsteps) for (int i = 0; i < 4; ++i) c->slab_pool.take(&ev[2 * i], &ev[2 * i + 1]);
            if (ev[0]) SLAB_HIP_TRY(hipEventRecord(ev[0], c->stream));
            const RK3Dev p = make_dev(c);
            SLAB_HIP_TRY(hipEventRecord(c->ev_dep, c->stream));
            if (ev[6]) SLAB_HIP_TRY(hipEventRecord(ev[6], c->stream));
            const int zi0 = has_below ? cb + 1 : 1, zi1 = has_above ? c->nzl - cb : c->nzl;
            if (has_interior) {
                if (has_below && has_above) launch_q23(c, p, c->stream, 1, cb, c->nzl - cb + 1, c->nzl);
                else if (has_below) launch_q23(c, p, c->stream, 1, cb, 1, 0);
                else launch_q23(c, p, c->stream, c->nzl - cb + 1, c->nzl, 1, 0);
            }
            else launch_step_range(c, p, c->stream, 1, c->nzl);
            if (ev[7]) SLAB_HIP_TRY(hipEventRecord(ev[7], c->stream));
            if (hipGetLastError() != hipSuccess) { set_error("lbmpm_rk3d_step_slab: kernel launch failed"); return fail(LBMPM_ERR_HIP); }
            if (ev[4]) SLAB_HIP_TRY(hipEventRecord(ev[4], c->stream));
            RK3Dev q = p;
            q.fin = c->fB; q.pur_in = c->purB; q.first = 0;
#ifdef LBMPM_DEV
            const int skip = c->dbg;
#else
            constexpr int skip = 0;
#endif
            if (!(skip & 1)) rk3dq_face_pack<<<fgrid, fblock, 0, c->stream>>>(q, c->send_up, c->send_dn, has_below, has_above);
            if (has_interior) {
                SLAB_HIP_TRY(hipEventRecord(c->ev_dep, c->stream));
                SLAB_HIP_TRY(hipStreamWaitEvent(c->aux, c->ev_dep, 0));
            }
            const double *from_below = c->recv_below, *from_above = c->recv_above;
            if (own_tx) {
                if (!(skip & 2)) { const int rc = c->tx.exchange(c->stream, c->send_up, c->send_dn, &from_below, &from_above); if (rc != LBMPM_OK) return fail(rc); }
            }
            else if (!(skip & 2) && exchange(user, 0) != 0) { set_error("lbmpm_rk3d_step_slab: the exchange callback failed"); return fail(LBMPM_ERR_STATE); }
            if (has_interior) {
                hipStream_t ist = (skip & 8) ? c->stream : c->aux;
                if (ev[2]) SLAB_HIP_TRY(hipEventRecord(ev[2], ist));
                launch_step_range(c, p, ist, zi0, zi1);
                if (ev[3]) SLAB_HIP_TRY(hipEventRecord(ev[3], ist));
                SLAB_HIP_TRY(hipEventRecord(c->ev_done, ist));
            }
            if (!(skip & 4)) {
                rk3dq_face_unpack<<<fgrid, fblock, 0, c->stream>>>(q, c->fB, c->purB, from_below, from_above, has_below, has_above);
                rk3dq_halo_phi<<<fgrid, fblock, 0, c->stream>>>(q, from_below, from_above, has_below, has_above);
                slabtx::launch_flag_store(c->stream, c->beat_dev, (unsigned long long)(c->steps + 1));
            }
            if (hipGetLastError() != hipSuccess) { set_error("lbmpm_rk3d_step_slab: face kernel launch failed"); return fail(LBMPM_ERR_HIP); }
            if (ev[5]) SLAB_HIP_TRY(hipEventRecord(ev[5], c->stream));
            if (has_interior) SLAB_HIP_TRY(hipStreamWaitEvent(c->stream, c->ev_done, 0));
            finish_step(c);
            c->halo_valid = !(skip & 6);
            if (ev[1]) SLAB_HIP_TRY(hipEventRecord(ev[1], c->stream));
        }
        return LBMPM_OK;
    }
#undef SLAB_HIP_TRY
    for (int64_t k = 0; k < nsteps; ++k) {
        hipEvent_t ev[8] = {nullptr, nullptr, nullptr, nullptr, nullptr, nullptr, nullptr, nullptr};
        if (k < tsteps) for (int i = 0; i < 4; ++i) c->slab_pool.take(&ev[2 * i], &ev[2 * i + 1]);
        if (ev[0]) LBMPM_HIP_TRY(hipEventRecord(ev[0], c->stream));
        int rc = LBMPM_OK;
        if (nb) rc = collide_interior_ev(c, ev[2], ev[3]);
        if (rc != LBMPM_OK) return rc;
        if (ev[4]) LBMPM_HIP_TRY(hipEventRecord(ev[4], c->stream));
        auto abandon = [&](int code) {
            if (c->interior_pending) { (void)hipStreamSynchronize(c->aux); c->interior_pending = false; }
            return code;
        };
        if (nb && c->streamed) {
            rc = lbmpm_rk3d_pack_halo(c);
            if (rc == LBMPM_OK && exchange(user, 0) != 0) { set_error("lbmpm_rk3d_step_slab: the exchange callback failed (populations)"); rc = LBMPM_ERR_STATE; }
            if (rc == LBMPM_OK) rc = lbmpm_rk3d_unpack_halo(c, has_below, has_above);
            if (rc != LBMPM_OK) return abandon(rc);
        }
        rc = lbmpm_rk3d_phase_field(c, 0);
        if (rc != LBMPM_OK) return abandon(rc);
        if (nb && exchange(user, 1) != 0) { set_error("lbmpm_rk3d_step_slab: the exchange callback failed (phase field)"); return abandon(LBMPM_ERR_STATE); }
        if (ev[5]) LBMPM_HIP_TRY(hipEventRecord(ev[5], c->stream));
        rc = collide_boundary_ev(c, ev[6], ev[7]);
        if (rc != LBMPM_OK) return rc;
        if (ev[1]) LBMPM_HIP_TRY(hipEventRecord(ev[1], c->stream));
    }
    return LBMPM_OK;
}

extern "C" int lbmpm_rk3d_slab_timing(lbmpm_rk3d *c, double *out)
{
    LBMPM_REQUIRE(c && out, "lbmpm_rk3d_slab_timing: null argument");
    LBMPM_HIP_TRY(hipStreamSynchronize(c->stream));
    if (c->aux) LBMPM_HIP_TRY(hipStreamSynchronize(c->aux));
    for (int i = 0; i < 5; ++i) out[i] = 0.;
    const int64_t n = c->slab_timed_steps;
    if (n <= 0) return LBMPM_OK;
    const bool has_interior = c->aux && !(c->variant == 1 || c->nzl < 2 * c->boundary + 1) &&
                              (c->cfg.z_offset > 0 || c->cfg.z_offset + c->cfg.nz_local < c->cfg.nz_global);
// ... 164 lines not shown
        return LBMPM_ERR_STATE;
    }
    switch (field) {
        case LBMPM_RK3D_PHI: src = c->phi; break;
        case LBMPM_RK3D_RHO_R: case LBMPM_RK3D_RHO_B: case LBMPM_RK3D_VX: case LBMPM_RK3D_VY: case LBMPM_RK3D_VZ:
            if (!c->diag) { set_error("field %d needs lbmpm_rk3d_phase_field(ctx, 1) first", field); return LBMPM_ERR_STATE; }
            src = c->diag + (size_t)(field - LBMPM_RK3D_RHO_R) * c->vol;
            break;
        default:
            set_error("lbmpm_rk3d_get_field: unknown field id %d", field);
            return LBMPM_ERR_INVALID;
    }
    std::vector<double> h(c->vol);
    LBMPM_HIP_TRY(hipMemcpyAsync(h.data(), src, c->vol * sizeof(double), hipMemcpyDeviceToHost, c->stream));
    LBMPM_HIP_TRY(hipStreamSynchronize(c->stream));
    const size_t hp = (size_t)c->nx * c->ny;
    for (int z = 0; z < c->nzl; ++z)
        for (int y = 0; y < c->ny; ++y)
            for (int x = 0; x < c->nx; ++x) {
                const size_t s = (size_t)z * hp + (size_t)y * c->nx + x;
                out[s] = c->h_domain[s] == 1 ? h[(size_t)(z + 1) * c->plane2 + (size_t)y * c->pitch + x] : 0.0;
            }
    return LBMPM_OK;
}

extern "C" int lbmpm_rk3d_storage_info(lbmpm_rk3d *c, int64_t *out)
{
    LBMPM_REQUIRE(c && out, "lbmpm_rk3d_storage_info: null argument");
    out[0] = c->q23 ? QS : 2 * Q; out[1] = c->nfluid; out[2] = 0;
    if (c->q23) {
        LBMPM_HIP_TRY(hipSetDevice(c->cfg.device));
        LBMPM_HIP_TRY(hipStreamSynchronize(c->stream));
        std::vector<uint32_t> f((size_t)(c->nzl + 2) * c->ny * c->nseg);
        LBMPM_HIP_TRY(hipMemcpy(f.data(), c->purA, f.size() * sizeof(uint32_t), hipMemcpyDeviceToHost));
        const size_t per = (size_t)c->ny * c->nseg;
        for (size_t r = per; r < per * (size_t)(c->nzl + 1); ++r)
            if (f[r] & 3u) out[2] += c->h_rowpop[r];
    }
    out[3] = c->q23 ? 2 * Q * 8 * out[1] + 64 * (out[1] - out[2]) : 2 * 2 * Q * 8 * out[1];
    return LBMPM_OK;
}

extern "C" int lbmpm_rk3d_debug_trace(lbmpm_rk3d *c, unsigned long long *out, int64_t nblocks)
{
#ifndef LBMPM_DEV
    LBMPM_REQUIRE(false, "lbmpm_rk3d_debug_trace: this library was built without -DLBMPM_DEV (per-workgroup time stamps exist in development builds only: tools/dev/devlib.py)");
#endif
    LBMPM_REQUIRE(c && out && c->trace && nblocks * 32 <= (1 << 22), "lbmpm_rk3d_debug_trace: tracing is off (LBMPM_RK3D_TRACE) or too many workgroups");
    LBMPM_HIP_TRY(hipDeviceSynchronize());
    LBMPM_HIP_TRY(hipMemcpy(out, c->trace, (size_t)nblocks * 32, hipMemcpyDeviceToHost));
    return LBMPM_OK;
}

extern "C" int lbmpm_rk3d_debug_plane(lbmpm_rk3d *c, int comp, int zl, double *out)
{
    LBMPM_REQUIRE(c && out && c->q23 && zl >= 0 && zl <= c->nzl + 1 && comp >= 0 && comp <= 24, "lbmpm_rk3d_debug_plane: q23 storage, plane 0..nzl+1, comp 0..24");
    LBMPM_HIP_TRY(hipSetDevice(c->cfg.device));
    LBMPM_HIP_TRY(hipStreamSynchronize(c->stream));
    if (c->aux) LBMPM_HIP_TRY(hipStreamSynchronize(c->aux));
    const size_t n = (size_t)c->nx * c->ny;
    if (comp == 24) {
        std::vector<uint32_t> f((size_t)c->ny * c->nseg);
        LBMPM_HIP_TRY(hipMemcpy(f.data(), c->purA + (size_t)zl * c->ny * c->nseg, f.size() * sizeof(uint32_t), hipMemcpyDeviceToHost));
        for (size_t i = 0; i < f.size(); ++i) out[i] = (double)f[i];
        return LBMPM_OK;
    }
    if (comp == 23) {
        std::vector<double> h(c->plane2);
        LBMPM_HIP_TRY(hipMemcpy(h.data(), c->phi + (size_t)zl * c->plane2, h.size() * sizeof(double), hipMemcpyDeviceToHost));
        for (int y = 0; y < c->ny; ++y) for (int x = 0; x < c->nx; ++x) out[(size_t)y * c->nx + x] = h[(size_t)y * c->pitch + x];
        return LBMPM_OK;
    }
    double *d = nullptr;
    LBMPM_HIP_TRY(hipMalloc(reinterpret_cast<void **>(&d), n * sizeof(double)));
    const RK3Dev p = make_dev(c);
    rk3dq_debug_plane<<<dim3(c->nseg, (c->ny + BY3 - 1) / BY3), dim3(BX3, BY3), 0, c->stream>>>(p, c->fA, zl, comp, d);
    hipError_t e = hipMemcpyAsync(out, d, n * sizeof(double), hipMemcpyDeviceToHost, c->stream);
    if (e == hipSuccess) e = hipStreamSynchronize(c->stream);
    (void)hipFree(d);
    if (e != hipSuccess) { set_error("lbmpm_rk3d_debug_plane: %s", hipGetErrorString(e)); return LBMPM_ERR_HIP; }
    return LBMPM_OK;
}

extern "C" int64_t lbmpm_rk3d_num_fluid_nodes(const lbmpm_rk3d *c) { return c ? c->nfluid : 0; }
extern "C" int64_t lbmpm_rk3d_steps_done(const lbmpm_rk3d *c) { return c ? c->steps : 0; }
extern "C" int64_t lbmpm_rk3d_device_bytes(const lbmpm_rk3d *c) { return c ? c->bytes : 0; }
extern "C" const char *lbmpm_rk3d_dominant_kernel(const lbmpm_rk3d *c) { return !c ? "" : (c->variant == 1 ? "rk3d_collide" : (c->q23 ? "rk3dq_fused" : (c->compact ? "rk3dc_fused" : "rk3d_fused"))); }
```

### openlbmpm_amd/csrc/rk3dq.h

```cpp

constexpr int QS = 23;
constexpr unsigned CELLB = QS * 8u;
constexpr int QLINE = 16;
constexpr int SR = 12, SC = 68;
constexpr int SCOMP = SR * SC;
constexpr int SSLOT = 4 * SCOMP;

typedef const unsigned long long __attribute__((address_space(4))) *const_u64_ptr;
__device__ __forceinline__ unsigned long long pstart_of(const RK3Dev &p, int zl) { return ((const_u64_ptr)p.pstart)[zl]; }

struct PlaneAddrQ {
    const char *base;
    unsigned off[3], cnt[3];
};

__device__ __forceinline__ PlaneAddrQ plane_addr_q(const RK3Dev &p, const double *f, int zl)
{
    PlaneAddrQ a;
    const unsigned long long p1 = pstart_of(p, zl), p2 = pstart_of(p, zl + 1);
    const unsigned long long p0 = zl > 0 ? pstart_of(p, zl - 1) : p1, p3 = zl <= p.nzl ? pstart_of(p, zl + 2) : p2;
    a.base = reinterpret_cast<const char *>(f) + (size_t)p0 * CELLB;
    a.cnt[0] = (unsigned)(p1 - p0); a.cnt[1] = (unsigned)(p2 - p1); a.cnt[2] = (unsigned)(p3 - p2);
    a.off[0] = 0u; a.off[1] = a.cnt[0] * CELLB; a.off[2] = a.off[1] + a.cnt[1] * CELLB;
    return a;
// ... 160 lines not shown
        for (int dx = -1; dx <= 1; ++dx) {
            const int i = DIRT[(1 - rz) * 9 + (1 - ry) * 3 + (1 - dx)];
            if (i <= 0) continue;
            unsigned j = 0;
            bool fl = true;
            if (!FIRST) row_cell<false>(t, dx, b, j, fl);
            const unsigned up = a.off[1 + rz] + (unsigned)i * a.cnt[1 + rz] * 8u + j * 8u;
            const unsigned back = a.off[1] + (unsigned)OPP[i] * a.cnt[1] * 8u + own8;
            g[i] = ldg(a.base, FIRST ? a.off[1] + (unsigned)i * a.cnt[1] * 8u + own8 : (fl ? up : back));
        }
    }
}

__device__ __forceinline__ void class_sums_pure(const double g[Q], bool red, Sums &S)
{
#pragma clang fp contract(off)
    constexpr int CZ[Q] = LBMPM_D3Q19_CZ;
    S.t0 = g[0]; S.tp = 0.; S.tm = 0.;
#pragma unroll
    for (int rz = -1; rz <= 1; ++rz)
#pragma unroll
        for (int ry = -1; ry <= 1; ++ry)
#pragma unroll
            for (int dx = -1; dx <= 1; ++dx) {
                const int i = DIRT[(1 - rz) * 9 + (1 - ry) * 3 + (1 - dx)];
                if (i <= 0) continue;
                if (CZ[i] == 0) S.t0 += g[i];
                else if (CZ[i] > 0) S.tp += g[i];
                else S.tm += g[i];
            }
    S.k0 = red ? S.t0 : 0.; S.kp = red ? S.tp : 0.; S.km = red ? S.tm : 0.;
    S.a0 = S.ap = S.am = 0.;
}

template <bool WITH_G, int PIN = -1>
__device__ __forceinline__ void bc_q(const RK3Dev &p, int zl, const Sums &S, double *g, double &rR, double &rho)
{
#pragma clang fp contract(off)
    const bool pin = PIN < 0 ? p.inletP != 0 : PIN == 1;
    const int zsg = p.z0 + source_plane(p, zl) - 1;
    const double r0 = S.k0 + S.a0, rp = S.kp + S.ap, rm = S.km + S.am;
    rR = (r0 + rp) + rm;
    rho = (S.t0 + S.tp) + S.tm;
    if (zsg == p.nzg - 2) {
        const double wR = r0 + 2. * rp, wT = S.t0 + 2. * S.tp;
        double J;
        if (pin) {
            rR = p.vzR;
            rho = p.vzR + p.vzB;
            J = wT - rho;
        } else {
            const double dR = wR / (1. + p.vzR), dB = (wT - wR) / (1. + p.vzB);
            rR = dR;
            rho = dR + dB;
            J = dR * p.vzR + dB * p.vzB;
        }
        if (WITH_G) {
            const double Nx = 0.5 * ((g[1] + g[7] + g[9]) - (g[2] + g[8] + g[10]));
            const double Ny = 0.5 * ((g[3] + g[7] + g[10]) - (g[4] + g[8] + g[9]));
            g[6] = g[5] - 1. / 3. * J;
            g[12] = g[11] - 1. / 6. * J + Nx;
            g[13] = g[14] - 1. / 6. * J - Nx;
            g[16] = g[15] - 1. / 6. * J + Ny;
            g[17] = g[18] - 1. / 6. * J - Ny;
        }
    }
    if (zsg == 1) {
        rR = p.rhoOutR;
        rho = p.rhoOutR + p.rhoOutB;
        if (WITH_G) {
            const double J = rho - (S.t0 + 2. * S.tm);
            const double Nx = 0.5 * ((g[1] + g[7] + g[9]) - (g[2] + g[8] + g[10]));
            const double Ny = 0.5 * ((g[3] + g[7] + g[10]) - (g[4] + g[8] + g[9]));
            g[5] = g[6] + 1. / 3. * J;
            g[11] = g[12] + 1. / 6. * J - Nx;
            g[14] = g[13] + 1. / 6. * J + Nx;
            g[15] = g[16] + 1. / 6. * J - Ny;
            g[18] = g[17] + 1. / 6. * J + Ny;
        }
    }
}
__device__ __forceinline__ double phi_q(double rR, double rho) { return (rR - (rho - rR)) / rho; }

template <bool FIRST, bool MRT, bool RAGGED, bool PIN = false>
__global__ __launch_bounds__(512, 1) void rk3dq_fused(RK3Dev p, int tilesX, int tilesY, int rows_per_xcd, int chunk_len, int z_first, int z_last,
                                                       int nchunks1, int z_first2, int z_last2,
                                                       unsigned *slotq)
{
    constexpr int TX = 64, TY = 8;
    using M = March<TX, TY>;
    using TR = TileRows<TY>;
    constexpr int CX[Q] = LBMPM_D3Q19_CX, CY[Q] = LBMPM_D3Q19_CY, CZ[Q] = LBMPM_D3Q19_CZ;
    __shared__ double sphi[M::RING][M::FY][M::FX];
    __shared__ double ssc[4 * SSLOT];
    __shared__ u32x4 srow[TR::SLOTS][TR::ROWS][6];
    __shared__ int sslot[2];
    const int tid = threadIdx.x;
    const int band_slots = (int)(gridDim.x >> 3);
    if (tid == 0 && !slotq) { sslot[0] = (int)(blockIdx.x & 7u); sslot[1] = (int)(blockIdx.x >> 3); }
    if (tid == 0 && slotq) {
        const int here = (int)(__builtin_amdgcn_s_getreg((3 << 11) | 20) & 7u);
        int band = -1, slot = 0;
        for (int k = 0; k < 8 && band < 0; ++k) {
            const int b = (here + k) & 7;
            const int q = (int)atomicAdd(&slotq[b], 1u);
            if (q < band_slots) { band = b; slot = q; }
        }
        sslot[0] = band; sslot[1] = slot;
    }
    __syncthreads();
    const int xcd = sslot[0], slot = sslot[1];
    if (xcd < 0) return;
#ifdef LBMPM_DEV
    const int bid = xcd + 8 * slot;
#endif
    const int tx = slot % tilesX, r = slot / tilesX, ty = xcd * rows_per_xcd + r % rows_per_xcd, chunk = r / rows_per_xcd;
    if (ty >= tilesY) return;
    const int wave = __builtin_amdgcn_readfirstlane(tid >> 6);
#ifdef LBMPM_DEV
    unsigned long long *trace = p.trace && z_last - z_first >= 8 ? p.trace + (size_t)bid * 4 : nullptr;
    if (trace && tid == 0) trace[0] = wall_clock64();
#endif
    int lx, ly, x, y, yo, hlx, hly, hx, hy, xrow, xc, xcol;
    bool own, has_own, has_rim, has_x, row_ok;
    TileRowsU<TY, true, RAGGED> rows_own{{srow, 0, 1}}, rows_rimrow{{srow, 0, 1}}, rows_xrow{{srow, 0, 1}};
    TileRowsU<TY, false, RAGGED> rows_rimcol{{srow, 0, 0}}, rows_xcol{{srow, 0, 0}};
    const int x0 = RAGGED ? seg_x0(tx, p.nx, tilesX) : tx * TX;
    const int tw = RAGGED ? seg_x0(tx + 1, p.nx, tilesX) - x0 : TX;
    const int twl = RAGGED ? (tx > 0 ? x0 - seg_x0(tx - 1, p.nx, tilesX) : p.nx - seg_x0(tilesX - 1, p.nx, tilesX)) : TX;
    auto set_geometry = [&](int t) {
        lx = t % TX; ly = t / TX;
        x = x0 + lx; y = ty * TY + ly;
        own = y < p.ny;
        yo = ring_coord(y, p.ny);
        row_ok = yo >= 0;
        has_own = row_ok && lx < tw;
        hlx = 0; hly = 0; hx = 0; hy = 0;
        has_rim = false;
        if (t < M::NH) {
            bool in_row = true;
            if (t < 2 * TX) { hlx = 1 + t % TX; hly = t < TX ? 0 : M::FY - 1; in_row = t % TX < tw; }
            else { const int k = t - 2 * TX; hlx = k < M::FY ? 0 : tw + 1; hly = k < M::FY ? k : k - M::FY; }
            hx = ring_coord(x0 + hlx - 1, p.nx);
            hy = ring_coord(ty * TY + hly - 1, p.ny);
            has_rim = hx >= 0 && hy >= 0 && in_row;
        }
        xrow = ly >= 3 && ly <= 6 ? (ly < 5 ? ly - 5 : ly + 3) : (lx >> 2) - 2;
        xc = lx & 3; xcol = ly == 7 ? (xc < 2 ? xc - 2 : tw + xc - 2) : lx;
        has_x = (ly >= 3 && ly <= 6) || (ly == 7 && lx < 4 * SR);
        rows_own.t.lrow = ly + 2;
        rows_rimrow.t.lrow = hly + 1;
        rows_rimcol.t.lrow = hly + 1; rows_rimcol.t.k = hlx == 0 ? 0 : 2;
        rows_xrow.t.lrow = xrow + 2;
        rows_xcol.t.lrow = xrow + 2; rows_xcol.t.k = xc < 2 ? 0 : 2;
    };
    set_geometry(tid);
    __shared__ unsigned sgeo[3][TX * TY];
    sgeo[0][tid] = (unsigned)lx | ((unsigned)ly << 6) | ((unsigned)hlx << 9) | ((unsigned)hly << 16) | ((unsigned)(xrow + 2) << 20) | ((unsigned)xc << 24) |
                   ((unsigned)own << 26) | ((unsigned)has_own << 27) | ((unsigned)has_rim << 28) | ((unsigned)has_x << 29) | ((unsigned)row_ok << 30);
    sgeo[1][tid] = ((unsigned)hx & 0xffffu) | ((unsigned)hy << 16);
    sgeo[2][tid] = ((unsigned)yo & 0xffffu) | ((unsigned)(xcol + 2) << 16);
    auto load_geometry = [&](int t) {
        const unsigned w0 = sgeo[0][t], w1 = sgeo[1][t], w2 = sgeo[2][t];
        lx = (int)(w0 & 63u); ly = (int)((w0 >> 6) & 7u);
        x = x0 + lx; y = ty * TY + ly;
        hlx = (int)((w0 >> 9) & 127u); hly = (int)((w0 >> 16) & 15u);
        xrow = (int)((w0 >> 20) & 15u) - 2; xc = (int)((w0 >> 24) & 3u);
        own = (w0 >> 26) & 1u; has_own = (w0 >> 27) & 1u; has_rim = (w0 >> 28) & 1u; has_x = (w0 >> 29) & 1u;
        row_ok = RAGGED ? (w0 >> 30) & 1u : has_own;
        hx = (int)(short)(w1 & 0xffffu); hy = (int)w1 >> 16;
        yo = (int)(short)(w2 & 0xffffu); xcol = (int)(w2 >> 16) - 2;
        rows_own.t.lrow = ly + 2;
        rows_rimrow.t.lrow = hly + 1;
        rows_rimcol.t.lrow = hly + 1; rows_rimcol.t.k = hlx == 0 ? 0 : 2;
        rows_xrow.t.lrow = xrow + 2;
        rows_xcol.t.lrow = xrow + 2; rows_xcol.t.k = xc < 2 ? 0 : 2;
    };
    const int za = chunk < nchunks1 ? z_first + chunk * chunk_len : z_first2 + (chunk - nchunks1) * chunk_len;
    const int zb = min(za + chunk_len - 1, chunk < nchunks1 ? z_last : z_last2);
    const int zl_gb = 1 - p.z0, zl_gt = p.nzg - p.z0;
    auto is_ghost = [&](int zl) { return zl == zl_gb || zl == zl_gt; };
    struct RowRec { u32x4 v; unsigned f0, f1, f2; };
    auto fetch_rows = [&](int zl) -> RowRec {
        RowRec q;
        q.v = u32x4{0u, 0u, 0u, 0u}; q.f0 = 0u; q.f1 = ~0u; q.f2 = ~0u;
        if (tid < TR::ROWS * 6 && zl >= 0 && zl <= p.nzl + 1) {
            const int row = tid / 6, k = tid % 6;
            int yy = (ty * TY - 2 + row) % p.ny;
            if (yy < 0) yy += p.ny;
            int sg = tx - 1 + (k >> 1);
            sg = sg < 0 ? sg + p.nseg : (sg >= p.nseg ? sg - p.nseg : sg);
            const unsigned rr = ((unsigned)zl * (unsigned)p.ny + (unsigned)yy) * (unsigned)p.nseg + (unsigned)sg;
            q.v = (k & 1) ? p.seg2[rr] : p.seg[rr];
            if (k & 1) {
                q.f0 = p.pur_in[rr];
                if (k == 3) {
                    const int sl = tx > 0 ? tx - 1 : p.nseg - 1, sr = tx + 1 < p.nseg ? tx + 1 : 0;
                    q.f1 = p.pur_in[rr - sg + sl]; q.f2 = p.pur_in[rr - sg + sr];
                }
            }
        }
        return q;
    };
    auto put_rows = [&](int zl, const RowRec &q) {
        if (tid < TR::ROWS * 6) {
            u32x4 v = q.v;
            if (tid & 1) { v.z = q.f0; v.w = q.f0 & q.f1 & q.f2; }
            const_cast<u32x4 &>(srow[zl & (TR::SLOTS - 1)][tid / 6][tid % 6]) = v;
        }
    };
    auto row_flag = [&](int zl, int lrow, int k) -> unsigned { return srow[zl & (TR::SLOTS - 1)][lrow][2 * k + 1].z; };
    struct SRec { double2 a, b; bool ok; };
    auto load_s = [&](int zl, unsigned j) -> SRec {
        const unsigned long long p0 = pstart_of(p, zl);
        const unsigned cnt = (unsigned)(pstart_of(p, zl + 1) - p0);
        const char *s = reinterpret_cast<const char *>(p.fin) + (size_t)p0 * CELLB + (size_t)cnt * (Q * 8u) + (size_t)j * 32u;
        SRec v;
        v.a = *reinterpret_cast<const double2 *>(s); v.b = *reinterpret_cast<const double2 *>(s + 16);
        v.ok = true;
        return v;
    };
    auto const_s = [&](unsigned flag) -> SRec {
        SRec v;
        v.a.x = (flag & 1u) ? 1. : 0.; v.a.y = 0.; v.b.x = 0.; v.b.y = 0.; v.ok = true;
        return v;
    };
    auto fetch_s = [&](int zl, SRec &e0, SRec &e1) {
        e0.ok = false; e1.ok = false;
        if (zl < 0 || zl > p.nzl + 1) return;
        {
            const RowTab t = rows_own(zl, 0);
            const unsigned fg = (unsigned)__builtin_amdgcn_readfirstlane((int)row_flag(zl, ly + 2, 1));
            if (bit_of<true>(t.m, (unsigned)lx)) e0 = fg ? const_s(fg) : load_s(zl, t.first + bits_below<true>(t.m, (unsigned)lx));
        }
        if (wave >= 3 && wave <= 6) {
            const RowTab t = rows_xrow(zl, 0);
            const unsigned fg = (unsigned)__builtin_amdgcn_readfirstlane((int)row_flag(zl, xrow + 2, 1));
            if (bit_of<true>(t.m, (unsigned)lx)) e1 = fg ? const_s(fg) : load_s(zl, t.first + bits_below<true>(t.m, (unsigned)lx));
        } else if (wave == 7) {
            if (has_x) {
                const RowTab t = rows_xcol(zl, 0);
                const unsigned fg = row_flag(zl, xrow + 2, xc < 2 ? 0 : 2);
                const unsigned bb = xc < 2 ? (unsigned)(twl - 2) + (unsigned)xc : (unsigned)xc - 2u;
                if (bit_of<false>(t.m, bb)) e1 = fg ? const_s(fg) : load_s(zl, t.first + bits_below<false>(t.m, bb));
            }
        }
    };
    auto put_s = [&](int zl, const SRec &e0, const SRec &e1) {
        double *sl = ssc + (zl & 3) * SSLOT;
        if (e0.ok) {
            double *d = sl + (ly + 2) * SC + lx + 2;
            d[0] = e0.a.x; d[SCOMP] = e0.a.y; d[2 * SCOMP] = e0.b.x; d[3 * SCOMP] = e0.b.y;
        }
        if (wave >= 3 && e1.ok) {
            double *d = sl + (xrow + 2) * SC + xcol + 2;
            d[0] = e1.a.x; d[SCOMP] = e1.a.y; d[2 * SCOMP] = e1.b.x; d[3 * SCOMP] = e1.b.y;
        }
    };
    auto purity = [&](int zp, int row_lo, int row_hi) -> int {
        unsigned c = 3u;
        for (int dz = -1; dz <= 1; ++dz)
            for (int rr = row_lo - 1; rr <= row_hi + 1; ++rr) c &= srow[(zp + dz) & (TR::SLOTS - 1)][rr + 2][3].w;
// ... 129 lines not shown
            else if (ghost_n) { if (has_own && zn == zl_gt) ph = sphi[z & (M::RING - 1)][ly + 1][lx + 1]; }
            else if (fl_raw) {
                Sums S;
                const int pc = purity(zn, ly, ly);
                mixed_n = pc == 0;
                if (pc != 0) class_sums_pure(raw, (pc & 1) != 0, S);
                else class_sums<FIRST, true>(p, rows_own, lds_scal(zn, ly, lx), zn, (unsigned)lx, raw, S);
                bc_q<true, PIN ? 1 : 0>(p, zn, S, raw, rRn, rhon);
                ph = phi_q(rRn, rhon);
            }
            if (has_own) {
                sphi[zn & (M::RING - 1)][ly + 1][lx + 1] = ph;
                if (fill_gb) sphi[(zn - 1) & (M::RING - 1)][ly + 1][lx + 1] = ph;
            }
#pragma unroll
            for (int i = 0; i < Q; ++i) { ft[i] = cur[i]; cur[i] = raw[i]; }
            rR = rRn; rho = rhon; jz = j_raw; mixed_w = mixed_n;
        }
        const bool padzz = padz;
        padz = pad_raw;
        PH_MARK(1)
        put_s(z + 3, e0, e1);
        __builtin_amdgcn_s_waitcnt(LBMPM_WAIT_VMCNT0);
        PH_MARK(2)
        if (z + 2 <= zb + 1) issue(z + 2);
        else { fl_raw = false; pad_raw = false; }
        staged = fetch_rows(z + 6);
        PH_MARK(3)
        __syncthreads();
        PH_MARK(4)
        const bool live = z >= za && !is_ghost(z);
        const bool active = live && fluid && own;
        if (__ballot(active) == 0ull) {
            pulls_landed();
            if (live && own && lx == 0) p.pur_out[row_index(p, z, y, tx)] = 3u;
        } else if (active) {
            LBMPM_TAKEN;
            double ax = 0., ay = 0., az = 0., dx = 0., dy = 0., dz = 0.;
#pragma unroll
            for (int i = 1; i < Q; ++i) {
                const double ph = sphi[(z + CZ[i]) & (M::RING - 1)][ly + 1 + CY[i]][lx + 1 + CX[i]];
                if (i < 7) {
                    if (CX[i] != 0) ax = CX[i] > 0 ? ax + ph : ax - ph;
                    if (CY[i] != 0) ay = CY[i] > 0 ? ay + ph : ay - ph;
                    if (CZ[i] != 0) az = CZ[i] > 0 ? az + ph : az - ph;
                } else {
                    if (CX[i] != 0) dx = CX[i] > 0 ? dx + ph : dx - ph;
                    if (CY[i] != 0) dy = CY[i] > 0 ? dy + ph : dy - ph;
                    if (CZ[i] != 0) dz = CZ[i] > 0 ? dz + ph : dz - ph;
                }
            }
            const double gx = 3. * wq(1) * ax + 3. * wq(7) * dx, gy = 3. * wq(1) * ay + 3. * wq(7) * dy, gz = 3. * wq(1) * az + 3. * wq(7) * dz;
            if (__builtin_amdgcn_readfirstlane((int)mixed_z))
                collide_store<2, MRT, true>(p, reinterpret_cast<char *>(p.fout) + (size_t)pz0 * CELLB, (unsigned)(pz1 - pz0) * 8u, jzz * 8u, true, ft, rRz,
                                            rhoz - rRz, gx, gy, gz, p.pur_out + row_index(p, z, y, tx));
            else
                collide_store<2, MRT>(p, reinterpret_cast<char *>(p.fout) + (size_t)pz0 * CELLB, (unsigned)(pz1 - pz0) * 8u, jzz * 8u, true, ft, rRz, rhoz - rRz,
                                      gx, gy, gz, p.pur_out + row_index(p, z, y, tx));
        }
        if (live && padzz) {
            char *pl = reinterpret_cast<char *>(p.fout) + (size_t)pz0 * CELLB;
            const unsigned stride = (unsigned)(pz1 - pz0) * 8u;
#pragma unroll
            for (int i = 0; i < Q; ++i) stg(pl + (size_t)i * stride, jzz * 8u, 0.);
        }
#pragma unroll
        for (int i = 0; i < Q; ++i) asm volatile("" : "+v"(raw[i]));
        fluid = fluidn;
        PH_MARK(5)
    }
#undef PH_MARK
#if defined(LBMPM_DEV) && defined(LBMPM_PHASES)
    if (p.trace && (tid & 63) == 0 && bid < 4096) {
        unsigned long long *o = p.trace + (1u << 18) + ((size_t)bid * 8 + (size_t)wave) * 8;
        for (int k = 0; k < 6; ++k) o[k] = ph_acc[k];
        o[6] = (unsigned long long)(zb - za + 1);
    }
#endif
#ifdef LBMPM_DEV
    if (trace && tid == 0) trace[2] = wall_clock64();
#endif
}

__global__ __launch_bounds__(BX3 *BY3) void rk3dq_init_rest(RK3Dev p, const double *rho_r, const double *rho_b, double *f, uint32_t *pur)
{
    const int sg = blockIdx.x, x = LBMPM_SEG_LANE_X(p, sg, (int)threadIdx.x), y = blockIdx.y * BY3 + threadIdx.y, zl = blockIdx.z + 1;
    if (y >= p.ny) return;
    const bool fluid = x >= 0 && (p.flags[(size_t)zl * p.plane2 + (size_t)y * p.pitch + x] & 1);
    double a = 0., b = 0.;
    if (fluid) {
        const GlobalRows rows{p, sg, y};
        const RowTab t = rows(zl, 0);
        const unsigned j = t.first + bits_below<false>(t.m, threadIdx.x);
        const size_t sd = ((size_t)(zl - 1) * p.ny + y) * p.nx + x;
        a = rho_r[sd]; b = rho_b[sd];
        const unsigned long long p0 = pstart_of(p, zl);
        const size_t cnt = (size_t)(pstart_of(p, zl + 1) - p0);
        double *pl = f + (size_t)p0 * QS;
        for (int i = 0; i < Q; ++i) pl[(size_t)i * cnt + j] = wq(i) * (a + b);
        double *s = pl + (size_t)Q * cnt + (size_t)j * 4;
        s[0] = a / (a + b); s[1] = 0.; s[2] = 0.; s[3] = 0.;
    }
    const unsigned code = (__ballot(fluid && b != 0.) == 0ull ? 1u : 0u) | (__ballot(fluid && a != 0.) == 0ull ? 2u : 0u);
    if (threadIdx.x == 0) pur[row_index(p, zl, y, sg)] = code;
}

__global__ __launch_bounds__(BX3 *BY3) void rk3dq_phase_field(RK3Dev p, int zl0)
{
    const int sg = blockIdx.x, x = LBMPM_SEG_LANE_X(p, sg, (int)threadIdx.x), y = blockIdx.y * BY3 + threadIdx.y, zl = blockIdx.z + zl0;
    if (y >= p.ny || x < 0) return;
    const size_t idx = (size_t)zl * p.plane2 + (size_t)y * p.pitch + x;
    if (!(p.flags[idx] & 1)) return;
    const int zs = source_plane_x(p, zl);
    const unsigned b = threadIdx.x;
    double g[Q], rR, rho;
    unsigned j;
    Sums S;
    const GlobalRows rows{p, sg, y};
    if (p.first) {
        pull_q<true, false>(p, rows, zs, b, g, j);
        class_sums<true, false>(p, rows, glb_scal(p, plane_addr_q(p, p.fin, zs), j, zs, sg, y), zs, b, g, S);
    } else {
        pull_q<false, false>(p, rows, zs, b, g, j);
        class_sums<false, false>(p, rows, glb_scal(p, plane_addr_q(p, p.fin, zs), j, zs, sg, y), zs, b, g, S);
    }
    bc_q<true>(p, p.conv && p.z0 + zl - 1 <= 2 ? zs : zl, S, g, rR, rho);
    p.phi[idx] = phi_q(rR, rho);
    if (p.diag) {
        constexpr int CX[Q] = LBMPM_D3Q19_CX, CY[Q] = LBMPM_D3Q19_CY, CZ[Q] = LBMPM_D3Q19_CZ;
        double mx = 0., my = 0., mz = 0.;
#pragma unroll
        for (int i = 0; i < Q; ++i) { mx += (double)CX[i] * g[i]; my += (double)CY[i] * g[i]; mz += (double)CZ[i] * g[i]; }
        p.diag[idx] = rR; p.diag[p.vol + idx] = rho - rR;
        p.diag[2 * p.vol + idx] = mx / rho; p.diag[3 * p.vol + idx] = my / rho; p.diag[4 * p.vol + idx] = mz / rho;
    }
}

__global__ __launch_bounds__(256) void rk3dq_conv_phi(RK3Dev p, int zs)
{
    const size_t k = (size_t)blockIdx.x * blockDim.x + threadIdx.x;
    if (k >= p.plane2 || !(p.flags[(size_t)zs * p.plane2 + k] & 1)) return;
    const double v = p.phi[(size_t)zs * p.plane2 + k];
    for (int zl = zs - 3; zl < zs; ++zl) p.phi[(size_t)zl * p.plane2 + k] = v;
}

template <bool FIRST, bool MRT>
__global__ __launch_bounds__(BX3 *BY3) void rk3dq_conv_collide(RK3Dev p, int zs)
{
    constexpr int CX[Q] = LBMPM_D3Q19_CX, CY[Q] = LBMPM_D3Q19_CY, CZ[Q] = LBMPM_D3Q19_CZ;
    const int sg = blockIdx.x, x = LBMPM_SEG_LANE_X(p, sg, (int)threadIdx.x), y = blockIdx.y * BY3 + threadIdx.y, zl = zs - 1 - (int)blockIdx.z;
    if (y >= p.ny) return;
    const bool fluid = x >= 0 && (p.flags[(size_t)zl * p.plane2 + (size_t)y * p.pitch + x] & 1);
    if (__ballot(fluid) == 0ull) {
        if (threadIdx.x == 0) p.pur_out[row_index(p, zl, y, sg)] = 3u;
        return;
    }
    if (!fluid) return;
    const GlobalRows rows{p, sg, y};
    const unsigned b = threadIdx.x;
    double g[Q], rR, rho;
    unsigned js;
    Sums S;
    pull_q<FIRST, false>(p, rows, zs, b, g, js);
    class_sums<FIRST, false>(p, rows, glb_scal(p, plane_addr_q(p, p.fin, zs), js, zs, sg, y), zs, b, g, S);
    bc_q<true>(p, zs, S, g, rR, rho);
    double gx = 0., gy = 0., gz = 0.;
// ... 134 lines not shown
```

### openlbmpm_amd/rk3d.py

```python
import ctypes as C

import numpy as np

from . import _lib
from ._lib import F64P, U8P, RK3DConfig, check
from .slab import partition_z, partition_z_balanced, neighbour_exchange, local_exchange, DeviceBuffer

FIELDS = dict(phi=0, rhoR=1, rhoB=2, vx=3, vy=4, vz=5)
BUF = dict(f_send_up=0, f_send_down=1, f_recv_below=2, f_recv_above=3,
           phi_send_up=4, phi_send_down=5, phi_recv_below=6, phi_recv_above=7)

DEFAULT_PARAMS = dict(AkR=7.0e-3, AkB=7.0e-3, beta=1.0, tauR=1.0, tauB=1.0, SolidRhoR=0.7, SolidRhoB=0.0,
                      velocityZR=0.0, velocityZB=-1.0e-4, densityRL=1.0e-8, densityBL=1.0, relax="SRT",
                      recolor_axis=0.0, recolor_diag=0.0,
                      inlet="Neumann", densityRH=1.0e-8, densityBH=1.0,
                      outlet="Dirichlet")


class RK3DSlab:

    def __init__(self, is_domain_global, z0, nzl, params=None, device=0):
        L = _lib.lib()
        p = dict(DEFAULT_PARAMS); p.update(params or {})
        unknown = set(p) - set(DEFAULT_PARAMS)
# ... 142 lines not shown
        check(self._L.lbmpm_rk3d_ipc_init(self._h, blob), "lbmpm_rk3d_ipc_init")
        return blob.raw

    def ipc_connect(self, blob_below, blob_above):
        keep = [C.create_string_buffer(b, _lib.IPC_BLOB_BYTES) if b is not None else None for b in (blob_below, blob_above)]
        check(self._L.lbmpm_rk3d_ipc_connect(self._h, keep[0], keep[1]), "lbmpm_rk3d_ipc_connect")

    @staticmethod
    def rccl_unique_id(librccl_path=None):
        idb = C.create_string_buffer(_lib.RCCL_ID_BYTES)
        check(_lib.lib().lbmpm_rccl_unique_id(idb, librccl_path.encode() if librccl_path else None), "lbmpm_rccl_unique_id")
        return idb.raw

    def rccl_connect(self, unique_id, rank, nranks, librccl_path=None):
        idb = C.create_string_buffer(unique_id, _lib.RCCL_ID_BYTES)
        check(self._L.lbmpm_rk3d_rccl_connect(self._h, idb, int(rank), int(nranks), librccl_path.encode() if librccl_path else None),
              "lbmpm_rk3d_rccl_connect")

    def transport_disconnect(self):
        check(self._L.lbmpm_rk3d_transport_disconnect(self._h), "lbmpm_rk3d_transport_disconnect")

    @property
    def transport(self):
        v = C.c_int(0)
        k = self._L.lbmpm_rk3d_transport_kind(self._h, C.byref(v))
        return {0: "callback", 1: "ipc (copy engine + %s)" % ("stream value operations" if v.value else "one-lane flag kernels"), 2: "rccl"}[k]

    def halo_exchange(self):
        check(self._L.lbmpm_rk3d_halo_exchange(self._h), "lbmpm_rk3d_halo_exchange")

    def transport_probe(self, rounds=6):
        check(self._L.lbmpm_rk3d_transport_probe(self._h, int(rounds)), "lbmpm_rk3d_transport_probe")

    def transport_probe_result(self):
        v = C.c_int64(-1)
        check(self._L.lbmpm_rk3d_transport_probe_result(self._h, C.byref(v)), "lbmpm_rk3d_transport_probe_result")
        return int(v.value)

    def ipc_release_waits(self):
        check(self._L.lbmpm_rk3d_ipc_release_waits(self._h), "lbmpm_rk3d_ipc_release_waits")

    def slab_timing(self):
        out = (C.c_double * 5)()
        check(self._L.lbmpm_rk3d_slab_timing(self._h, out), "lbmpm_rk3d_slab_timing")
        return dict(step_ms=out[0], interior_ms=out[1], exchange_chain_ms=out[2], boundary_ms=out[3], steps=int(out[4]))

    def step_single(self, n):
        check(self._L.lbmpm_rk3d_step(self._h, int(n)), "lbmpm_rk3d_step")

    def step_timed(self, n):
        a, b = C.c_double(0), C.c_double(0)
        check(self._L.lbmpm_rk3d_step_timed(self._h, int(n), C.byref(a), C.byref(b)), "step_timed")
        return a.value, b.value

    def sync(self, deadline_s=None):
        if deadline_s is None:
            check(self._L.lbmpm_rk3d_sync(self._h), "sync")
        else:
            check(self._L.lbmpm_rk3d_sync_deadline(self._h, float(deadline_s)), "lbmpm_rk3d_sync_deadline")

    def get(self, name):
        out = np.empty((self.nzl, self.ny, self.nx), dtype=np.float64)
        check(self._L.lbmpm_rk3d_get_field(self._h, FIELDS[name], out.ctypes.data_as(F64P)), "get_field(%s)" % name)
        return out

    @property
    def num_fluid_nodes(self):
        return int(self._L.lbmpm_rk3d_num_fluid_nodes(self._h))

    @property
    def device_bytes(self):
        return int(self._L.lbmpm_rk3d_device_bytes(self._h))

    def debug_plane(self, comp, zl):
        n = self.ny * ((self.nx + 63) // 64 if comp == 24 else self.nx)
        out = np.zeros(n, dtype=np.float64)
        check(self._L.lbmpm_rk3d_debug_plane(self._h, int(comp), int(zl), out.ctypes.data_as(F64P)), "lbmpm_rk3d_debug_plane")
        return out.reshape(self.ny, -1)

    def storage_info(self):
        out = (C.c_int64 * 4)()
        check(self._L.lbmpm_rk3d_storage_info(self._h, out), "lbmpm_rk3d_storage_info")
        return dict(doubles_per_cell=int(out[0]), fluid_cells=int(out[1]), cells_in_flagged_rows=int(out[2]), bytes_per_step=int(out[3]))

    @property
    def steps_done(self):
        return int(self._L.lbmpm_rk3d_steps_done(self._h))

    @property
    def dominant_kernel(self):
        return self._L.lbmpm_rk3d_dominant_kernel(self._h).decode()

    @property
    def one_exchange(self):
        return self.dominant_kernel == "rk3dq_fused"


def _torch_librccl():
    import os
    try:
        import torch
        p = os.path.join(os.path.dirname(torch.__file__), "lib", "librccl.so")
        return p if os.path.exists(p) else None
    except ImportError:
        return None


class RK3DCluster:

    def __init__(self, is_domain_global, k, params=None, device=0):
        nz = is_domain_global.shape[0]
        self.parts = partition_z(nz, k)
        import torch
        self.slabs = [RK3DSlab(is_domain_global, z0, n, params, device) for z0, n in self.parts]
        self.stream = torch.cuda.Stream(device)
        self._torch = torch
        for s in self.slabs:
            s.use_torch_stream(self.stream)
        self.k = k

    def set_density(self, rhoR, rhoB):
        for s, (z0, n) in zip(self.slabs, self.parts):
            s.set_density(rhoR[z0:z0 + n], rhoB[z0:z0 + n])

    def set_macro(self, rhoR, rhoB, vx=None, vy=None, vz=None):
        cut = lambda a, z0, n: None if a is None else a[z0:z0 + n]
        for s, (z0, n) in zip(self.slabs, self.parts):
            s.set_macro(*[cut(a, z0, n) for a in (rhoR, rhoB, vx, vy, vz)])

    def set_pdf(self, fR, fB, post_collision=True):
        for s, (z0, n) in zip(self.slabs, self.parts):
            s.set_pdf(fR[z0:z0 + n], fB[z0:z0 + n], post_collision)

    def get_pdf(self):
        got = [s.get_pdf() for s in self.slabs]
        return np.concatenate([g[0] for g in got], axis=0), np.concatenate([g[1] for g in got], axis=0)

    def get_state(self):
        got = [s.get_state() for s in self.slabs]
        return np.concatenate([g[0] for g in got], axis=0), got[0][1]

    def set_state(self, state, steps=0, post_collision=True):
        for s, (z0, n) in zip(self.slabs, self.parts):
            s.set_state(state[z0:z0 + n], steps, post_collision)

    def _exchange(self, kind):
        S = self.slabs
        if S[0].buffer(kind + "_send_up") is None:
            return
        local_exchange([s.buffer(kind + "_send_up") for s in S], [s.buffer(kind + "_send_down") for s in S],
                       [s.buffer(kind + "_recv_below") for s in S], [s.buffer(kind + "_recv_above") for s in S])

    def _halo_f(self):
        for s in self.slabs:
            s.pack()
        self._exchange("f")
        for r, s in enumerate(self.slabs):
            s.unpack(r > 0, r + 1 < self.k)

    def step(self, n):
        with self._torch.cuda.stream(self.stream):
            for _ in range(int(n)):
                for s in self.slabs:
                    s.collide_interior()
                if self.slabs[0].post_collision or self.slabs[0].one_exchange:
                    self._halo_f()
# ... 259 lines not shown
```

Before: 13660.

## Add deep-interior fast path splitting z-chunks into pure-phase and general kernels

Adds a planning kernel that, per tile and z-chunk, scans the purity bitmaps to find runs of planes at the chunk ends where the whole neighbourhood is single-phase fluid. Those planes are handled by a new lighter kernel, rk3dq_deep, which skips the general recoloring work and computes the colour gradient from neighbour flags. The fused kernel now reads a per-slot plane range from the plan and shrinks or skips its chunk. This costs an extra plan launch and a second kernel launch per step, and adds complexity in tracking which planes each kernel owns. Boundary-only launches keep the general path.

```diff
diff --git a/include/lbmpm.h b/include/lbmpm.h
--- a/include/lbmpm.h
+++ b/include/lbmpm.h
@@ -232,6 +232,7 @@
 int lbmpm_rk3d_buffer(lbmpm_rk3d *ctx, int which, void **device_ptr, int64_t *bytes);
 int lbmpm_rk3d_get_field(lbmpm_rk3d *ctx, int field, double *out);
 int lbmpm_rk3d_storage_info(lbmpm_rk3d *ctx, int64_t *out);
+int lbmpm_rk3d_deep_stats(lbmpm_rk3d *ctx, int64_t *out);
 int lbmpm_rk3d_debug_trace(lbmpm_rk3d *ctx, unsigned long long *out, int64_t nblocks);
 int lbmpm_rk3d_debug_plane(lbmpm_rk3d *ctx, int comp, int zl, double *out);
 int64_t lbmpm_rk3d_num_fluid_nodes(const lbmpm_rk3d *ctx);
diff --git a/openlbmpm_amd/_lib.py b/openlbmpm_amd/_lib.py
--- a/openlbmpm_amd/_lib.py
+++ b/openlbmpm_amd/_lib.py
@@ -162,6 +162,7 @@
     "lbmpm_rk3d_dominant_kernel": (C.c_char_p, [C.c_void_p]),
     "lbmpm_rk3d_device_bytes": (C.c_int64, [C.c_void_p]),
     "lbmpm_rk3d_storage_info": (C.c_int, [C.c_void_p, I64P]),
+    "lbmpm_rk3d_deep_stats": (C.c_int, [C.c_void_p, I64P]),
     "lbmpm_rk3d_debug_trace": (C.c_int, [C.c_void_p, C.c_void_p, C.c_int64]),
     "lbmpm_rk3d_debug_plane": (C.c_int, [C.c_void_p, C.c_int, C.c_int, F64P]),
     "lbmpm_rk3dcsf_create": (C.c_int, [C.POINTER(RK3DCSFConfig), U8P, C.POINTER(C.c_void_p)]),
diff --git a/openlbmpm_amd/csrc/rk3d.hip b/openlbmpm_amd/csrc/rk3d.hip
--- a/openlbmpm_amd/csrc/rk3d.hip
+++ b/openlbmpm_amd/csrc/rk3d.hip
@@ -48,6 +48,7 @@
     int halo_lo;
     int conv;
     int inletP;
+    int deep;
 };
 
 struct Cell { unsigned o[3][3]; };
@@ -1007,7 +1008,13 @@
     bool q23 = false;
     unsigned long long *trace = nullptr;
     unsigned *slotq = nullptr;
+    static constexpr unsigned SLOTQ_WORDS = 16;
     unsigned slot_launches = 0;
+    bool deep = true;
+    int2 *plan = nullptr;
+    size_t plan_cap = 0;
+    struct DeepRec { const unsigned *q; int64_t total; };
+    std::vector<DeepRec> deep_now, deep_last;
     unsigned long long *probe_bad = nullptr;
     slabtx::Transport tx;
     bool halo_valid = false;
@@ -1061,6 +1068,7 @@
     p.trace = c->trace;
 #endif
     p.pur_in = c->purA; p.pur_out = c->purB;
+    p.deep = c->deep ? 1 : 0;
     return p;
 }
 
@@ -1137,6 +1145,7 @@
     if (const char *e = getenv("LBMPM_RK3D_LAYOUT")) if (!strcmp(e, "dense")) c->compact = false;
     c->q23 = c->compact && c->tile == 0;
     if (const char *e = getenv("LBMPM_RK3D_STORAGE")) if (atoi(e) == 38) c->q23 = false;
+    if (const char *e = getenv("LBMPM_RK3D_DEEP")) if (atoi(e) == 0) c->deep = false;
     if (!c->q23 && c->nx % 64 != 0) c->compact = false;
     if (c->conv && !c->q23) c->compact = false;
     if (c->q23 && (c->nx > 32767 || c->ny > 32767)) {
@@ -1243,7 +1252,11 @@
 #ifdef LBMPM_DEV
         if (getenv("LBMPM_RK3D_XCC") && atoi(getenv("LBMPM_RK3D_XCC")) == 0) by_xcc = false;
 #endif
-        if (by_xcc) TRY_RC(dev_alloc(c, &c->slotq, 2 * 4096 * 8));
+        if (by_xcc) TRY_RC(dev_alloc(c, &c->slotq, 2 * 4096 * lbmpm_rk3d::SLOTQ_WORDS));
+        if (by_xcc && c->deep) {
+            c->plan_cap = (size_t)8 * c->nseg * ((((size_t)c->ny + 7) / 8 + 7) / 8) * ((size_t)c->nzl / 8 + 2);
+            TRY_RC(dev_alloc(c, &c->plan, c->plan_cap));
+        }
         LBMPM_REQUIRE((size_t)(c->nzl + 2) * c->ny * c->nseg < ((size_t)1 << 31), "rk3d: more than 2^31 row segments in one slab");
         TRY_RC(dev_alloc(c, &c->purA, (size_t)(c->nzl + 2) * c->ny * c->nseg));
         TRY_RC(dev_alloc(c, &c->purB, (size_t)(c->nzl + 2) * c->ny * c->nseg));
@@ -1283,7 +1296,7 @@
     if (c->probe_bad) (void)hipFree(c->probe_bad);
     if (c->beat_host) (void)hipHostFree(c->beat_host);
     if (c->wd_stream) (void)hipStreamDestroy(c->wd_stream);
-    for (void *ptr : {(void *)c->seg, (void *)c->seg2, (void *)c->pstart, (void *)c->flags, (void *)c->solidnbr, (void *)c->fA, (void *)c->fB, (void *)c->purA, (void *)c->purB, (void *)c->trace, (void *)c->slotq, (void *)c->phi, (void *)c->diag,
+    for (void *ptr : {(void *)c->seg, (void *)c->seg2, (void *)c->pstart, (void *)c->flags, (void *)c->solidnbr, (void *)c->fA, (void *)c->fB, (void *)c->purA, (void *)c->purB, (void *)c->trace, (void *)c->slotq, (void *)c->plan, (void *)c->phi, (void *)c->diag,
                       (void *)c->send_up, (void *)c->send_dn, (void *)c->recv_below, (void *)c->recv_above})
         if (ptr) (void)hipFree(ptr);
     c->pool.destroy();
@@ -1593,12 +1606,16 @@
     const int nchunks1 = (n1 + chunk_len - 1) / chunk_len;
     const int nchunks2 = n2 > 0 ? (n2 + chunk_len - 1) / chunk_len : 0;
     const dim3 grid((unsigned)(8 * tilesX * rpx * (nchunks1 + nchunks2))), block(512);
-    unsigned *q = nullptr;
-    if (c->slotq) {
+    auto slice = [&]() -> unsigned * {
+        if (!c->slotq) return nullptr;
         const unsigned n = c->slot_launches++, ring = (n / 4096u) & 1u, i = n % 4096u;
-        if (i == 2048u) (void)hipMemsetAsync(c->slotq + (size_t)(ring ^ 1u) * 4096u * 8u, 0, 4096u * 8u * sizeof(unsigned), st);
-        q = c->slotq + ((size_t)ring * 4096u + i) * 8u;
-    }
+        if (i == 2048u) (void)hipMemsetAsync(c->slotq + (size_t)(ring ^ 1u) * 4096u * lbmpm_rk3d::SLOTQ_WORDS, 0, 4096u * lbmpm_rk3d::SLOTQ_WORDS * sizeof(unsigned), st);
+        return c->slotq + ((size_t)ring * 4096u + i) * lbmpm_rk3d::SLOTQ_WORDS;
+    };
+    unsigned *q = slice();
+    const bool deep = p.deep && !p.first && n2 == 0 && q && c->plan && (size_t)grid.x <= c->plan_cap;
+    if (deep) rk3dq_deep_plan<<<grid, block, 0, st>>>(p, tilesX, tilesY, rpx, chunk_len, z_first, z_last, c->plan, q + 8);
+    c->deep_now.push_back({deep ? q : nullptr, (int64_t)tilesX * tilesY * (n1 + n2)});
     auto go = [&](auto first, auto mrt) {
         constexpr bool F = decltype(first)::value, M = decltype(mrt)::value;
         auto launch = [&](auto ragged, auto pin) {
@@ -1608,7 +1625,19 @@
         dispatch2(c->nx % 64 != 0, p.inletP != 0, launch);
     };
     dispatch2(p.first != 0, p.mrt != 0, go);
-}
+    if (deep) {
+        unsigned *q2 = slice();
+        auto go2 = [&](auto mrt, auto ragged) {
+            constexpr bool M = decltype(mrt)::value, R = decltype(ragged)::value;
+            const dim3 grid2(2 * grid.x), block2(256);
+            if (p.inletP) rk3dq_deep<M, R, true><<<grid2, block2, 0, st>>>(p, tilesX, tilesY, rpx, chunk_len, z_first, z_last, c->plan, q2);
+            else rk3dq_deep<M, R, false><<<grid2, block2, 0, st>>>(p, tilesX, tilesY, rpx, chunk_len, z_first, z_last, c->plan, q2);
+        };
+        dispatch2(p.mrt != 0, c->nx % 64 != 0, go2);
+    }
+}
+
+RK3Dev general_only(RK3Dev p) { p.deep = 0; return p; }
 
 void launch_step_range(lbmpm_rk3d *c, const RK3Dev &p, hipStream_t st, int z_first, int z_last)
 {
@@ -1647,6 +1676,8 @@
 {
     std::swap(c->fA, c->fB);
     std::swap(c->purA, c->purB);
+    c->deep_last.swap(c->deep_now);
+    c->deep_now.clear();
     c->streamed = true;
     c->steps += 1;
     c->halo_valid = false;
@@ -1708,6 +1739,7 @@
     }
     const int cb = c->boundary;
     RK3Dev p = make_dev(c);
+    p.deep = 0;
     if (e0) LBMPM_HIP_TRY(hipEventRecord(e0, c->stream));
     launch_step_range(c, p, c->stream, 1, cb);
     launch_step_range(c, p, c->stream, c->nzl - cb + 1, c->nzl);
@@ -2007,9 +2039,9 @@
                 SLAB_HIP_TRY(hipStreamWaitEvent(c->aux, c->ev_dep, 0));
                 if (ev[6]) SLAB_HIP_TRY(hipEventRecord(ev[6], c->aux));
                 const int zi0 = has_below ? cb + 1 : 1, zi1 = has_above ? c->nzl - cb : c->nzl;
-                if (has_below && has_above) launch_q23(c, p, c->aux, 1, cb, c->nzl - cb + 1, c->nzl);
-                else if (has_below) launch_q23(c, p, c->aux, 1, cb, 1, 0);
-                else launch_q23(c, p, c->aux, c->nzl - cb + 1, c->nzl, 1, 0);
+                if (has_below && has_above) launch_q23(c, general_only(p), c->aux, 1, cb, c->nzl - cb + 1, c->nzl);
+                else if (has_below) launch_q23(c, general_only(p), c->aux, 1, cb, 1, 0);
+                else launch_q23(c, general_only(p), c->aux, c->nzl - cb + 1, c->nzl, 1, 0);
                 if (ev[7]) SLAB_HIP_TRY(hipEventRecord(ev[7], c->aux));
                 RK3Dev q = p;
                 q.fin = c->fB; q.pur_in = c->purB; q.first = 0;
@@ -2047,9 +2079,9 @@
             if (ev[6]) SLAB_HIP_TRY(hipEventRecord(ev[6], c->stream));
             const int zi0 = has_below ? cb + 1 : 1, zi1 = has_above ? c->nzl - cb : c->nzl;
             if (has_interior) {
-                if (has_below && has_above) launch_q23(c, p, c->stream, 1, cb, c->nzl - cb + 1, c->nzl);
-                else if (has_below) launch_q23(c, p, c->stream, 1, cb, 1, 0);
-                else launch_q23(c, p, c->stream, c->nzl - cb + 1, c->nzl, 1, 0);
+                if (has_below && has_above) launch_q23(c, general_only(p), c->stream, 1, cb, c->nzl - cb + 1, c->nzl);
+                else if (has_below) launch_q23(c, general_only(p), c->stream, 1, cb, 1, 0);
+                else launch_q23(c, general_only(p), c->stream, c->nzl - cb + 1, c->nzl, 1, 0);
             }
             else launch_step_range(c, p, c->stream, 1, c->nzl);
             if (ev[7]) SLAB_HIP_TRY(hipEventRecord(ev[7], c->stream));
@@ -2380,6 +2412,22 @@
     return LBMPM_OK;
 }
 
+extern "C" int lbmpm_rk3d_deep_stats(lbmpm_rk3d *c, int64_t *out)
+{
+    LBMPM_REQUIRE(c && out, "lbmpm_rk3d_deep_stats: null argument");
+    out[0] = 0; out[1] = 0;
+    if (c->deep_last.empty()) return LBMPM_OK;
+    LBMPM_HIP_TRY(hipSetDevice(c->cfg.device));
+    LBMPM_HIP_TRY(hipStreamSynchronize(c->stream));
+    if (c->aux) LBMPM_HIP_TRY(hipStreamSynchronize(c->aux));
+    for (const lbmpm_rk3d::DeepRec &r : c->deep_last) {
+        unsigned w[2] = {0u, (unsigned)r.total};
+        if (r.q) LBMPM_HIP_TRY(hipMemcpy(w, r.q + 8, sizeof w, hipMemcpyDeviceToHost));
+        out[0] += w[0]; out[1] += w[1];
+    }
+    return LBMPM_OK;
+}
+
 extern "C" int64_t lbmpm_rk3d_num_fluid_nodes(const lbmpm_rk3d *c) { return c ? c->nfluid : 0; }
 extern "C" int64_t lbmpm_rk3d_steps_done(const lbmpm_rk3d *c) { return c ? c->steps : 0; }
 extern "C" int64_t lbmpm_rk3d_device_bytes(const lbmpm_rk3d *c) { return c ? c->bytes : 0; }
diff --git a/openlbmpm_amd/csrc/rk3dq.h b/openlbmpm_amd/csrc/rk3dq.h
--- a/openlbmpm_amd/csrc/rk3dq.h
+++ b/openlbmpm_amd/csrc/rk3dq.h
@@ -266,6 +266,12 @@
 }
 __device__ __forceinline__ double phi_q(double rR, double rho) { return (rR - (rho - rR)) / rho; }
 
+__device__ __forceinline__ void chunk_planes_of(int chunk, int chunk_len, int z_first, int z_last, int nchunks1, int z_first2, int z_last2, int &za, int &zb)
+{
+    za = chunk < nchunks1 ? z_first + chunk * chunk_len : z_first2 + (chunk - nchunks1) * chunk_len;
+    zb = min(za + chunk_len - 1, chunk < nchunks1 ? z_last : z_last2);
+}
+
 template <bool FIRST, bool MRT, bool RAGGED, bool PIN = false>
 __global__ __launch_bounds__(512, 1) void rk3dq_fused(RK3Dev p, int tilesX, int tilesY, int rows_per_xcd, int chunk_len, int z_first, int z_last,
                                                        int nchunks1, int z_first2, int z_last2,
@@ -281,6 +287,7 @@
     __shared__ int sslot[2];
     const int tid = threadIdx.x;
     const int band_slots = (int)(gridDim.x >> 3);
+    __shared__ int splan[2];
     if (tid == 0 && !slotq) { sslot[0] = (int)(blockIdx.x & 7u); sslot[1] = (int)(blockIdx.x >> 3); }
     if (tid == 0 && slotq) {
         const int here = (int)(__builtin_amdgcn_s_getreg((3 << 11) | 20) & 7u);
@@ -292,13 +299,23 @@
         }
         sslot[0] = band; sslot[1] = slot;
     }
+    if (tid == 0 && sslot[0] >= 0) {
+        int a, b;
+        chunk_planes_of(sslot[1] / tilesX / rows_per_xcd, chunk_len, z_first, z_last, nchunks1, z_first2, z_last2, a, b);
+        if (slotq) {
+            const int2 *plan = *reinterpret_cast<const int2 *const *>(slotq + 10);
+            if (plan) { const int2 e = plan[sslot[0] * band_slots + sslot[1]]; a = e.x; b = e.y; }
+        }
+        splan[0] = a; splan[1] = b;
+        if (a > b) sslot[0] = -1;
+    }
     __syncthreads();
     const int xcd = sslot[0], slot = sslot[1];
     if (xcd < 0) return;
 #ifdef LBMPM_DEV
     const int bid = xcd + 8 * slot;
 #endif
-    const int tx = slot % tilesX, r = slot / tilesX, ty = xcd * rows_per_xcd + r % rows_per_xcd, chunk = r / rows_per_xcd;
+    const int tx = slot % tilesX, r = slot / tilesX, ty = xcd * rows_per_xcd + r % rows_per_xcd;
     if (ty >= tilesY) return;
     const int wave = __builtin_amdgcn_readfirstlane(tid >> 6);
 #ifdef LBMPM_DEV
@@ -360,8 +377,7 @@
         rows_xrow.t.lrow = xrow + 2;
         rows_xcol.t.lrow = xrow + 2; rows_xcol.t.k = xc < 2 ? 0 : 2;
     };
-    const int za = chunk < nchunks1 ? z_first + chunk * chunk_len : z_first2 + (chunk - nchunks1) * chunk_len;
-    const int zb = min(za + chunk_len - 1, chunk < nchunks1 ? z_last : z_last2);
+    const int za = __builtin_amdgcn_readfirstlane(splan[0]), zb = __builtin_amdgcn_readfirstlane(splan[1]);
     const int zl_gb = 1 - p.z0, zl_gt = p.nzg - p.z0;
     auto is_ghost = [&](int zl) { return zl == zl_gb || zl == zl_gt; };
     struct RowRec { u32x4 v; unsigned f0, f1, f2; };
@@ -657,6 +673,191 @@
 #endif
 }
 
+constexpr int DEEP_MIN = 8;
+constexpr int DEEP_CAP = 512;
+
+__global__ __launch_bounds__(512) void rk3dq_deep_plan(RK3Dev p, int tilesX, int tilesY, int rows_per_xcd, int chunk_len, int z_first, int z_last,
+                                                        int2 *plan, unsigned *stats)
+{
+    constexpr int TY = 8, ROWS = TY + 4;
+    __shared__ unsigned scol[DEEP_CAP + 4];
+    __shared__ unsigned long long selig[DEEP_CAP / 64];
+    const int tid = threadIdx.x, band = (int)(blockIdx.x & 7u), slot = (int)(blockIdx.x >> 3);
+    const int tx = slot % tilesX, r = slot / tilesX, ty = band * rows_per_xcd + r % rows_per_xcd, chunk = r / rows_per_xcd;
+    int ca, cb;
+    chunk_planes_of(chunk, chunk_len, z_first, z_last, 1 << 30, 1, 0, ca, cb);
+    int2 *out = plan + (size_t)band * (gridDim.x >> 3) + slot;
+    if (blockIdx.x == 0 && tid == 0) *reinterpret_cast<int2 **>(stats + 2) = plan;
+    if (ty >= tilesY || ca > cb) { if (tid == 0) *out = make_int2(ca, cb); return; }
+    const int n = cb - ca + 1, nd = min(n, DEEP_CAP), np = nd + 4;
+    for (int k = tid; k < np; k += 512) scol[k] = 3u;
+    __syncthreads();
+    for (int idx = tid; idx < np * ROWS; idx += 512) {
+        const int k = idx / ROWS, row = idx % ROWS, zl = ca - 2 + k;
+        unsigned w = 0u;
+        if (zl >= 0 && zl <= p.nzl + 1) {
+            int yy = (ty * TY - 2 + row) % p.ny;
+            if (yy < 0) yy += p.ny;
+            const unsigned r0 = ((unsigned)zl * (unsigned)p.ny + (unsigned)yy) * (unsigned)p.nseg;
+            const int sl = tx > 0 ? tx - 1 : p.nseg - 1, sr = tx + 1 < p.nseg ? tx + 1 : 0;
+            w = p.pur_in[r0 + tx] & p.pur_in[r0 + sl] & p.pur_in[r0 + sr];
+        }
+        atomicAnd(&scol[k], w);
+    }
+    __syncthreads();
+    {
+        const int z = ca + tid, zg = p.z0 + z - 1;
+        unsigned c = 0u;
+        if (tid < nd && z - 2 >= 1 && z - 2 > p.halo_lo && z + 2 <= p.nzl && zg - 2 >= 2 && zg + 2 <= p.nzg - 3)
+            c = scol[tid] & scol[tid + 1] & scol[tid + 2] & scol[tid + 3] & scol[tid + 4];
+        const unsigned long long m = __ballot(c != 0u);
+        if ((tid & 63) == 0) selig[tid >> 6] = m;
+    }
+    __syncthreads();
+    if (tid == 0) {
+        int lo = 0, hi = 0;
+        while (lo < nd && ((selig[lo >> 6] >> (lo & 63)) & 1ull)) ++lo;
+        if (lo < n && n == nd) while (hi < nd && ((selig[(nd - 1 - hi) >> 6] >> ((nd - 1 - hi) & 63)) & 1ull)) ++hi;
+        if (lo < DEEP_MIN) lo = 0;
+        if (hi < DEEP_MIN) hi = 0;
+        *out = make_int2(ca + lo, cb - hi);
+        if (lo + hi) atomicAdd(&stats[0], (unsigned)(lo + hi));
+        atomicAdd(&stats[1], (unsigned)n);
+    }
+}
+
+typedef const u32x4 __attribute__((address_space(4))) *const_u32x4_ptr;
+typedef const uint32_t __attribute__((address_space(4))) *const_u32_ptr;
+struct Rows9 {
+    RowTab t[3][3];
+    int zc;
+    __device__ __forceinline__ RowTab operator()(int zl, int ry) const
+    {
+        const int d = zl - zc;
+        return d < 0 ? t[0][ry + 1] : (d == 0 ? t[1][ry + 1] : t[2][ry + 1]);
+    }
+};
+
+template <bool MRT, bool RAGGED, bool PIN>
+__global__ __launch_bounds__(256) void rk3dq_deep(RK3Dev p, int tilesX, int tilesY, int rows_per_xcd, int chunk_len, int z_first, int z_last,
+                                                   const int2 *plan, unsigned *slotq)
+{
+    constexpr int TY = 8;
+    constexpr int CX[Q] = LBMPM_D3Q19_CX, CY[Q] = LBMPM_D3Q19_CY, CZ[Q] = LBMPM_D3Q19_CZ;
+    __shared__ int sslot[2];
+    const int tid = threadIdx.x;
+    const int band_slots = (int)(gridDim.x >> 3);
+    if (tid == 0) {
+        const int here = (int)(__builtin_amdgcn_s_getreg((3 << 11) | 20) & 7u);
+        int band = -1, slot = 0;
+        for (int k = 0; k < 8 && band < 0; ++k) {
+            const int b = (here + k) & 7;
+            const int q = (int)atomicAdd(&slotq[b], 1u);
+            if (q < band_slots) { band = b; slot = q; }
+        }
+        sslot[0] = band; sslot[1] = slot;
+    }
+    __syncthreads();
+    const int xcd = __builtin_amdgcn_readfirstlane(sslot[0]), slot2 = __builtin_amdgcn_readfirstlane(sslot[1]);
+    if (xcd < 0) return;
+    const int slot = slot2 >> 1;
+    const int tx = slot % tilesX, r = slot / tilesX, ty = xcd * rows_per_xcd + r % rows_per_xcd, chunk = r / rows_per_xcd;
+    if (ty >= tilesY) return;
+    const int wave = __builtin_amdgcn_readfirstlane(tid >> 6) + 4 * (slot2 & 1);
+    const int yw = ty * TY + wave;
+    if (yw >= p.ny) return;
+    int ca, cb;
+    chunk_planes_of(chunk, chunk_len, z_first, z_last, 1 << 30, 1, 0, ca, cb);
+    const int2 gen = plan[(size_t)xcd * (band_slots >> 1) + slot];
+    const int ga = __builtin_amdgcn_readfirstlane(gen.x), gb = __builtin_amdgcn_readfirstlane(gen.y);
+    const unsigned lane = (unsigned)tid & 63u;
+    const int yr[3] = {yw > 0 ? yw - 1 : p.ny - 1, yw, yw + 1 < p.ny ? yw + 1 : 0};
+    const const_u32x4_ptr cseg = (const_u32x4_ptr)p.seg, cseg2 = (const_u32x4_ptr)p.seg2;
+    for (int end = 0; end < 2; ++end) {
+        const int da = end == 0 ? ca : max(gb + 1, ga), db = end == 0 ? min(ga - 1, cb) : cb;
+        if (da > db) continue;
+        double nxt[Q], cur[Q];
+#pragma unroll
+        for (int i = 0; i < Q; ++i) { nxt[i] = 0.; cur[i] = 0.; }
+        unsigned j_n = 0u, nb_n = 0u;
+        bool fl_n = false, pad_n = false;
+        for (int z = da - 1; z <= db; ++z) {
+            const unsigned jz = j_n, nb = nb_n;
+            const bool fluid = fl_n, padz = pad_n;
+#pragma unroll
+            for (int i = 0; i < Q; ++i) cur[i] = nxt[i];
+            fl_n = false; pad_n = false;
+            if (z < db) {
+                const int zl = z + 1;
+                Rows9 R;
+                R.zc = zl;
+#pragma unroll
+                for (int dz = 0; dz < 3; ++dz)
+#pragma unroll
+                    for (int ry = 0; ry < 3; ++ry) {
+                        const unsigned rr = (unsigned)__builtin_amdgcn_readfirstlane(
+                            (int)(((unsigned)(zl - 1 + dz) * (unsigned)p.ny + (unsigned)yr[ry]) * (unsigned)p.nseg + (unsigned)tx));
+                        R.t[dz][ry] = make_row<true, RAGGED>(cseg[rr], cseg2[rr]);
+                    }
+                const RowTab t = R.t[1][1];
+                fl_n = bit_of<true>(t.m, lane);
+                nb_n = 0u;
+                if (!fl_n) {
+                    const unsigned rank = bits_below<true>(~t.m, lane);
+                    pad_n = rank < t.pad;
+                    j_n = t.first + (unsigned)__popcll(t.m) + rank;
+                } else {
+                    pull_q<false, true, Rows9, false>(p, R, zl, lane, nxt, j_n);
+#pragma unroll
+                    for (int i = 1; i < Q; ++i) {
+                        unsigned jj;
+                        bool f;
+                        row_cell<true>(R.t[1 + CZ[i]][1 + CY[i]], CX[i], lane, jj, f);
+                        nb_n |= f ? 1u << i : 0u;
+                    }
+                }
+            }
+            if (z < da) continue;
+            const unsigned long long pz0 = pstart_of(p, z), pz1 = pstart_of(p, z + 1);
+            const unsigned frow = (unsigned)__builtin_amdgcn_readfirstlane((int)row_index(p, z, yw, tx));
+            const bool red = (((const_u32_ptr)p.pur_in)[frow] & 1u) != 0u;
+            if (__ballot(fluid) == 0ull) {
+                __builtin_amdgcn_s_waitcnt(LBMPM_WAIT_VMCNT0);
+                if (lane == 0u) p.pur_out[frow] = 3u;
+            } else if (fluid) {
+                Sums S;
+                double rR, rho;
+                class_sums_pure(cur, red, S);
+                bc_q<true, PIN ? 1 : 0>(p, z, S, cur, rR, rho);
+                const double pc = red ? 1. : -1.;
+                double ax = 0., ay = 0., az = 0., dx = 0., dy = 0., dz = 0.;
+#pragma unroll
+                for (int i = 1; i < Q; ++i) {
+                    const double ph = ((nb >> i) & 1u) ? pc : p.solidPhi;
+                    if (i < 7) {
+                        if (CX[i] != 0) ax = CX[i] > 0 ? ax + ph : ax - ph;
+                        if (CY[i] != 0) ay = CY[i] > 0 ? ay + ph : ay - ph;
+                        if (CZ[i] != 0) az = CZ[i] > 0 ? az + ph : az - ph;
+                    } else {
+                        if (CX[i] != 0) dx = CX[i] > 0 ? dx + ph : dx - ph;
+                        if (CY[i] != 0) dy = CY[i] > 0 ? dy + ph : dy - ph;
+                        if (CZ[i] != 0) dz = CZ[i] > 0 ? dz + ph : dz - ph;
+                    }
+                }
+                const double gx = 3. * wq(1) * ax + 3. * wq(7) * dx, gy = 3. * wq(1) * ay + 3. * wq(7) * dy, gz = 3. * wq(1) * az + 3. * wq(7) * dz;
+                collide_store<2, MRT>(p, reinterpret_cast<char *>(p.fout) + (size_t)pz0 * CELLB, (unsigned)(pz1 - pz0) * 8u, jz * 8u, true, cur, rR, rho - rR,
+                                      gx, gy, gz, p.pur_out + frow);
+            }
+            if (padz) {
+                char *pl = reinterpret_cast<char *>(p.fout) + (size_t)pz0 * CELLB;
+                const unsigned stride = (unsigned)(pz1 - pz0) * 8u;
+#pragma unroll
+                for (int i = 0; i < Q; ++i) stg(pl + (size_t)i * stride, jz * 8u, 0.);
+            }
+        }
+    }
+}
+
 __global__ __launch_bounds__(BX3 *BY3) void rk3dq_init_rest(RK3Dev p, const double *rho_r, const double *rho_b, double *f, uint32_t *pur)
 {
     const int sg = blockIdx.x, x = LBMPM_SEG_LANE_X(p, sg, (int)threadIdx.x), y = blockIdx.y * BY3 + threadIdx.y, zl = blockIdx.z + 1;
diff --git a/openlbmpm_amd/rk3d.py b/openlbmpm_amd/rk3d.py
--- a/openlbmpm_amd/rk3d.py
+++ b/openlbmpm_amd/rk3d.py
@@ -248,6 +248,11 @@
         out = (C.c_int64 * 4)()
         check(self._L.lbmpm_rk3d_storage_info(self._h, out), "lbmpm_rk3d_storage_info")
         return dict(doubles_per_cell=int(out[0]), fluid_cells=int(out[1]), cells_in_flagged_rows=int(out[2]), bytes_per_step=int(out[3]))
+
+    def deep_stats(self):
+        out = (C.c_int64 * 2)()
+        check(self._L.lbmpm_rk3d_deep_stats(self._h, out), "lbmpm_rk3d_deep_stats")
+        return int(out[0]), int(out[1])
 
     @property
     def steps_done(self):
```

Measured after the change: 10130. -25.9%, worse.
